# kohjingyu/gill

Hardware: AMD Instinct MI355X
Metric: 512x512 images/sec/node, OPT-6.7B+SD1.5 50-step (higher is better)
Workload: dtype bf16

## Files before the change

### gill_amd/_native.py

```python
from __future__ import annotations

import ctypes as C
import os
from typing import Dict, Iterable, List, Optional, Sequence, Tuple

import torch

_HERE = os.path.dirname(os.path.abspath(__file__))
LIB_PATH = os.environ.get("GILL_AMD_LIB") or os.path.join(_HERE, "libgill_amd.so")


class GillNativeError(RuntimeError):
  pass


class gill_tensor(C.Structure):
  _fields_ = [("name", C.c_char_p), ("data", C.c_void_p), ("dtype", C.c_int32), ("ndim", C.c_int32),
              ("shape", C.c_int64 * 4)]


class gill_opt_config(C.Structure):
  _fields_ = [(n, C.c_int32) for n in ("vocab_size", "hidden_size", "num_layers", "num_heads", "ffn_dim",
                                       "max_positions", "max_batch", "max_seq")]


class gill_mapper_config(C.Structure):
  _fields_ = [(n, C.c_int32) for n in ("in_dim", "out_dim", "hidden_dim", "num_heads", "ffn_dim", "num_enc_layers",
                                       "num_dec_layers", "num_input_tokens", "num_output_tokens", "max_batch")]


class gill_unet_config(C.Structure):
  _fields_ = [("in_channels", C.c_int32), ("out_channels", C.c_int32), ("block_out_channels", C.c_int32 * 4),
              ("layers_per_block", C.c_int32), ("cross_attention_dim", C.c_int32), ("num_heads", C.c_int32),
              ("norm_num_groups", C.c_int32), ("sample_size", C.c_int32), ("ctx_len", C.c_int32),
              ("max_batch", C.c_int32), ("heads_per_level", C.c_int32 * 4), ("v_prediction", C.c_int32),
              ("fp8_convs", C.c_int32)]


class gill_decode_rule(C.Structure):
  _fields_ = [("n_ret", C.c_int32), ("ret_ids", C.c_int32 * 16), ("n_gen", C.c_int32), ("gen_ids", C.c_int32 * 16),
              ("step", C.c_int32), ("min_word_tokens", C.c_int32), ("ret_eq_gen", C.c_int32),
              ("ret_scale", C.c_double), ("gen_scale", C.c_double), ("filter_value", C.c_double)]


class gill_decode_sampler(C.Structure):
  _fields_ = [("seed", C.c_uint64), ("draw", C.c_int32), ("row0", C.c_int32), ("temperature", C.c_double), ("top_p", C.c_double)]


class gill_clip_config(C.Structure):
  _fields_ = [(n, C.c_int32) for n in ("image_size", "patch_size", "hidden_size", "num_layers", "num_heads", "intermediate_size",
                                       "max_batch")]


class gill_clip_text_config(C.Structure):
  _fields_ = [(n, C.c_int32) for n in ("vocab_size", "hidden_size", "num_layers", "num_heads", "intermediate_size", "max_positions",
                                       "hidden_act", "max_batch")]


class gill_vae_config(C.Structure):
  _fields_ = [("latent_channels", C.c_int32), ("out_channels", C.c_int32), ("block_out_channels", C.c_int32 * 4),
              ("layers_per_block", C.c_int32), ("norm_num_groups", C.c_int32), ("latent_size", C.c_int32),
              ("scaling_factor", C.c_float), ("max_batch", C.c_int32)]


class gill_sd_sampler(C.Structure):
  _fields_ = [("kind", C.c_int32), ("steps_offset", C.c_int32), ("set_alpha_to_one", C.c_int32), ("eta", C.c_float)]


SD_ROW_DOUBLES = 12


_vp, _i, _f = C.c_void_p, C.c_int, C.c_float
SYMBOLS: Dict[str, Tuple[object, List[object]]] = {
  "gill_last_error": (C.c_char_p, []),
  "gill_version": (_i, []),
  "gill_opt_create": (_i, [C.POINTER(_vp), C.POINTER(gill_opt_config), C.POINTER(gill_tensor), _i]),
  "gill_opt_destroy": (None, [_vp]),
  "gill_opt_create_ex": (_i, [C.POINTER(_vp), C.POINTER(gill_opt_config), C.POINTER(gill_tensor), _i, _i]),
  "gill_opt_weight_mode": (_i, [_vp]),
  "gill_opt_decode_uses_w8": (_i, [_vp, _i]),
  "gill_opt_cached_uses_w8": (_i, [_vp, _i, _i, _i]),
  "gill_w8_max_rows": (_i, []),
  "gill_op_w8_quant": (_i, [_vp, _i, _i, _vp, _vp, _vp]),
  "gill_op_w8_dequant": (_i, [_vp, _vp, _i, _i, _i, _vp, _vp]),
  "gill_op_linear_w8": (_i, [_vp, _vp, _vp, _vp, _vp, _vp, _i, _i, _i, _i, _i, _i, _vp, _vp, _vp, _vp]),
  "gill_opt_embed": (_i, [_vp, _vp, _i, _vp, _vp]),
  "gill_opt_forward": (_i, [_vp, _vp, _i, _i, _vp, _vp]),
  "gill_opt_forward_cached": (_i, [_vp, _vp, _i, _i, _i, _vp, _vp]),
  "gill_opt_img_hidden": (_i, [_vp, _vp, C.POINTER(C.c_int32), _i, _i, _i, _vp, _vp, _vp]),
  "gill_opt_img_hidden_ex": (_i, [_vp, _vp, C.POINTER(C.c_int32), _i, _i, _i, _vp, _i, _vp, _vp, _vp]),
  "gill_opt_last_logits": (_i, [_vp, _vp, _i, _i, _vp, _vp]),
  "gill_opt_next_token": (_i, [_vp, _vp, _i, _i, C.POINTER(gill_decode_rule), _vp, _vp, _i, _i, _vp, _vp, _vp]),
  "gill_opt_pick_token": (_i, [_vp, _vp, _i, C.POINTER(gill_decode_rule), _vp, _i, _i, _vp, _vp, _vp]),
  "gill_opt_decode_logits": (_i, [_vp, _vp, _i, _i, C.POINTER(gill_decode_rule), _vp, _vp]),
  "gill_opt_filter_logits": (_i, [_vp, _vp, _vp, _i, C.c_double, C.c_double, C.c_double, _i, _vp]),
  "gill_opt_sample_token": (_i, [_vp, _vp, _i, _i, C.POINTER(gill_decode_rule), C.POINTER(gill_decode_sampler), _vp, _vp, _i, _i, _vp,
                                 _vp, _vp]),
  "gill_opt_draw_token": (_i, [_vp, _vp, _i, C.POINTER(gill_decode_rule), C.POINTER(gill_decode_sampler), _vp, _i, _i, _vp, _vp, _vp]),
  "gill_decode_uniforms": (_i, [C.c_uint64, C.c_int32, C.c_int32, C.c_int32, C.c_int32, C.POINTER(C.c_float)]),
  "gill_attention_decode": (_i, [_vp, _vp, _vp, _i, _vp, _vp, _vp, _vp, _i, _i, _i, _i, _vp, _vp]),
  "gill_attention_append": (_i, [_vp, _vp, _vp, _i, _vp, _vp, _vp, _vp, _i, _i, _i, _i, _i, _vp, _vp]),
  "gill_attention_extend": (_i, [_vp, _vp, _vp, _i, _vp, _vp, _vp, _vp, _vp, _i, _i, _i, _i, _i, _i, _vp, _vp]),
  "gill_opt_extend": (_i, [_vp, _vp, _vp, _vp, _i, _vp, _vp, _i, _i, _i, _i, _vp, _vp, _vp]),
  "gill_attention_fork_ws_bytes": (C.c_int64, [_i, _i, _i, _i]),
  "gill_attention_fork": (_i, [_vp, _vp, _vp, _i, _vp, _vp, _vp, _vp, _vp, _vp, _i, _i, _i, _i, _i, _i, _i, _vp, _vp, C.c_int64, _vp]),
  "gill_opt_score_candidates": (_i, [_vp, _vp, _vp, _vp, _i, _vp, _vp, _vp, _vp, _i, _i, _i, _i, _vp, _vp, _vp, _vp, _vp, _vp, _vp, _vp]),
  "gill_opt_set_kv_format": (_i, [_vp, _i]),
  "gill_opt_kv_format": (_i, [_vp]),
  "gill_opt_kv_bytes": (C.c_int64, [_vp]),
  "gill_attention_decode_kv8": (_i, [_vp, _vp, _vp, _i, _vp, _vp, _vp, _vp, _vp, _vp, _i, _i, _i, _i, _vp, _vp]),
  "gill_attention_extend_kv8": (_i, [_vp, _vp, _vp, _i, _vp, _vp, _vp, _vp, _vp, _vp, _vp, _i, _i, _i, _i, _i, _i, _vp, _vp]),
  "gill_opt_decode_step": (_i, [_vp, _vp, _vp, _i, _i, _vp, _vp]),
  "gill_opt_prefill_ids": (_i, [_vp, _vp, _i, _i, _vp, _i, _vp, _vp]),
  "gill_opt_next_token_ragged": (_i, [_vp, _vp, _i, C.POINTER(gill_decode_rule), _i, C.POINTER(gill_decode_sampler), _vp, _vp, _vp, _i, _vp,
                                      _vp]),
  "gill_opt_pick_token_ragged": (_i, [_vp, _vp, _i, C.POINTER(gill_decode_rule), _i, C.POINTER(gill_decode_sampler), _vp, _vp, _i, _vp, _vp]),
  "gill_clip_create": (_i, [C.POINTER(_vp), C.POINTER(gill_clip_config), C.POINTER(gill_tensor), _i]),
  "gill_clip_destroy": (None, [_vp]),
  "gill_clip_forward": (_i, [_vp, _vp, _i, _vp, _vp]),
  "gill_clip_preprocess_workspace": (_i, [C.POINTER(C.c_int64), _i, _i, C.POINTER(C.c_int64)]),
  "gill_clip_preprocess": (_i, [_vp, C.c_int64, C.POINTER(C.c_int64), _i, _i, _i, _vp, _vp, _vp, C.c_int64, _vp]),
  "gill_clip_resize_ksize": (_i, [_i, _i]),
  "gill_clip_resize_taps": (_i, [_i, _i, _i, _i, C.POINTER(C.c_int32), C.POINTER(C.c_int32), C.POINTER(C.c_int32), _i]),
  "gill_clip_text_create": (_i, [C.POINTER(_vp), C.POINTER(gill_clip_text_config), C.POINTER(gill_tensor), _i]),
  "gill_clip_text_destroy": (None, [_vp]),
  "gill_clip_text_forward": (_i, [_vp, _vp, _i, _i, _vp, _vp, _vp]),
  "gill_mapper_create": (_i, [C.POINTER(_vp), C.POINTER(gill_mapper_config), C.POINTER(gill_tensor), _i]),
  "gill_mapper_destroy": (None, [_vp]),
  "gill_mapper_forward": (_i, [_vp, _vp, _vp, _i, _i, _vp, _vp]),
  "gill_unet_create": (_i, [C.POINTER(_vp), C.POINTER(gill_unet_config), C.POINTER(gill_tensor), _i]),
  "gill_unet_destroy": (None, [_vp]),
  "gill_unet_forward": (_i, [_vp, _vp, C.POINTER(C.c_float), _vp, _i, _vp, _vp]),
  "gill_sd_denoise": (_i, [_vp, _vp, _vp, _i, _vp, _i, _i, _f, _vp, _vp]),
  "gill_vae_create": (_i, [C.POINTER(_vp), C.POINTER(gill_vae_config), C.POINTER(gill_tensor), _i]),
  "gill_vae_destroy": (None, [_vp]),
  "gill_vae_decode": (_i, [_vp, _vp, _i, _vp, _vp, _vp]),
  "gill_vae_encode": (_i, [_vp, _vp, _i, _vp, _vp, _vp, _vp]),
  "gill_sd_schedule_from": (_i, [_vp, _i, _i, _i, C.POINTER(C.c_float), C.POINTER(C.c_double), C.POINTER(C.c_double),
                                 C.POINTER(C.c_double)]),
  "gill_sd_denoise_from": (_i, [_vp, _vp, _vp, _vp, _i, _i, _vp, _vp, _i, _i, _f, _vp, _vp, _vp]),
  "gill_op_sd_sampler_run_from": (_i, [_vp, _i, _i, _i, _f, _vp, _vp, _vp, _vp, _i, C.c_int64, _vp, _vp, _vp]),
  "gill_sd_inpaint_prepare": (_i, [_vp, _vp, _i, _i, _i, _i, _vp, _vp, _vp]),
  "gill_sd_inpaint_keep": (_i, [_vp, _i, _i, _i, C.POINTER(C.c_double)]),
  "gill_sd_inpaint": (_i, [_vp, _vp, _vp, _vp, _i, _i, _vp, _vp, _vp, _vp, _i, _i, _f, _vp, _vp, _vp]),
  "gill_op_sd_inpaint_run": (_i, [_vp, _i, _i, _i, _f, _vp, _vp, _vp, _vp, _vp, _vp, _i, C.c_int64, C.c_int64, _vp, _vp, _vp]),
  "gill_op_conv3x3_ex": (_i, [_vp, _i, _vp, _i, _vp, _vp, _vp, _vp, _vp, _i, _i, _i, _i, _i, _i, _i, _i, _vp]),
  "gill_op_conv3x3_fp8": (_i, [_vp, _vp, _vp, _vp, _vp, _i, _i, _i, _i, _i, _i, _vp]),
  "gill_ret_index_create": (_i, [C.POINTER(_vp), _i, C.c_int64]),
  "gill_ret_index_destroy": (None, [_vp]),
  "gill_ret_index_add": (_i, [_vp, _vp, _i, C.c_int64, _i, _f, _vp]),
  "gill_ret_index_size": (C.c_int64, [_vp]),
  "gill_ret_index_rows": (_i, [_vp, C.c_int64, C.c_int64, _vp, _vp]),
  "gill_ret_index_search": (_i, [_vp, _vp, _i, _i, _i, _vp, _i, _f, _vp, _vp, _vp]),
  "gill_ret_index_slabs": (_i, [_vp, C.POINTER(C.c_int64), C.POINTER(C.c_int), C.POINTER(C.c_int64)]),
  "gill_pndm_schedule": (_i, [_i, C.POINTER(C.c_int32), C.POINTER(C.c_double)]),
  "gill_sd_denoise_ex": (_i, [_vp, _vp, _vp, _vp, _i, _vp, _i, _i, _f, _vp, _vp, _vp]),
  "gill_sd_schedule": (_i, [_vp, _i, _i, C.POINTER(C.c_float), C.POINTER(C.c_double), C.POINTER(C.c_double)]),
  "gill_op_sd_sampler_run": (_i, [_vp, _i, _i, _f, _vp, _vp, _vp, _i, C.c_int64, _vp, _vp, _vp]),
  "gill_coop_timeouts": (_i, []),
  "gill_op_gemm": (_i, [_vp, _vp, _vp, _vp, _vp, _i, _i, _i, _f, _i, _i, _i, _vp]),
  "gill_op_geglu": (_i, [_vp, _vp, _vp, _vp, _i, _i, _i, _vp]),
  "gill_op_conv3x3": (_i, [_vp, _i, _vp, _i, _vp, _vp, _vp, _vp, _vp, _i, _i, _i, _i, _i, _i, _i, _vp]),
  "gill_op_attention": (_i, [_vp, _vp, _vp, _vp, _i, _i, _i, _i, _i, _f, _i, _vp]),
  "gill_op_layernorm": (_i, [_vp, _i, _vp, _vp, _vp, _i, _i, _f, _vp]),
  "gill_op_groupnorm": (_i, [_vp, _i, _vp, _i, _i, _i, _i, _vp, _vp, _f, _i, _vp, _vp]),
  "gill_op_conv3x3_gn_stats": (_i, [_vp, _i, _vp, _i, _vp, _vp, _vp, _vp, _vp, _i, _vp, _i, _vp, _vp, _vp, _i, _i, _i, _i, _i, _i, _i,
                                    C.POINTER(C.c_int), C.POINTER(C.c_int), _vp]),
  "gill_op_gemm_gn_stats": (_i, [_vp, _vp, _vp, _vp, _vp, _vp, _i, _i, _i, _i, _i, _i, _i, C.POINTER(C.c_int), C.POINTER(C.c_int), _vp]),
  "gill_op_groupnorm_from_stats": (_i, [_vp, _i, _vp, _i, _i, _i, _i, _vp, _vp, _f, _i, _vp, _i, _i, _vp, _i, _i, _vp, _vp, _f, _vp]),
  "gill_op_conv3x3_gn": (_i, [_vp, _vp, _vp, _vp, _vp, _vp, _vp, _i, _f, _i, _vp, _vp, _vp, _i, _i, _i, _i, _i, _i, _i, _vp]),
  "gill_op_conv3x3_shortcut": (_i, [_vp, _i, _vp, _i, _vp, _vp, _vp, _i, _vp, _i, _vp, _vp, _i, _i, _i, _i, _i, _vp]),
  "gill_op_ffn_fused": (_i, [_vp, _vp, _vp, _vp, _vp, _vp, _vp, _vp, _vp, _vp, _vp, _vp, _i, _i, _vp, _vp, _vp, _vp]),
  "gill_op_geglu_fp8": (_i, [_vp, _vp, _vp, _vp, _vp, _vp, _i, _i, _i, _vp]),
  "gill_conv_fp8_kpad": (_i, [_i]),
  "gill_op_quant_fp8": (_i, [_vp, _f, C.c_int64, _vp, _vp]),
  "gill_op_conv_weight_quant_fp8": (_i, [_vp, _i, _i, _i, _f, _vp, _vp, _vp]),
  "gill_op_conv3x3_fp8_q": (_i, [_vp, _vp, _vp, _vp, _vp, _vp, _vp, _vp, _i, _vp, _i, _i, _i, _i, _i, _i, _i, _vp]),
  "gill_op_groupnorm_fp8": (_i, [_vp, _i, _vp, _i, _i, _i, _i, _vp, _vp, _f, _i, _f, _vp, _vp]),
  "gill_op_linear_weight_quant_fp8": (_i, [_vp, _i, _i, _f, _vp, _vp, _vp]),
  "gill_op_ln_quant_fp8": (_i, [_vp, _i, _i, _vp, _i, _i, _f, _f, _vp, _vp]),
  "gill_op_geglu_fp8_q": (_i, [_vp, _vp, _vp, _vp, _vp, _i, _i, _i, _vp]),
  "gill_op_lnproj": (_i, [_i, _vp, _vp, _vp, _vp, _vp, _vp, _vp, _vp, _vp, _vp, _i, _i, _vp]),
  "gill_op_cross_attention_folded": (_i, [_vp, _vp, _vp, _vp, _vp, _vp, _vp, _vp, _vp, _vp, _vp, _i, _i, _i, _i, _i, _i, _vp]),
  "gill_op_linear_rowstats": (_i, [_vp, _vp, _i, _vp, _vp, _vp, _vp, _vp, _i, C.POINTER(C.c_int), _i, _i, _i, _i, _vp]),
  "gill_op_ln_gemm": (_i, [_i, _vp, _vp, _i, _i, _vp, _vp, _vp, _vp, _vp, _vp, _vp, _vp, _i, _i, _i, _i, _i, _i, _i, _i, _vp]),
  "gill_op_vae_attention": (_i, [_vp, _vp, _vp, _vp, _vp, _vp, _vp, _vp, _i, _i, _i, C.POINTER(C.c_int), _vp]),
  "gill_op_row_softmax": (_i, [_vp, _i, _i, _vp]),
  "gill_op_conv_out": (_i, [_vp, _vp, _i, _vp, _vp, _i, _i, _i, _i, _i, _i, C.POINTER(C.c_int), _vp]),
  "gill_op_conv_in": (_i, [_vp, _vp, _i, _vp, _vp, _i, _i, _i, _i, _i, _vp, _i, _vp]),
  "gill_op_conv_in_wide": (_i, [_vp, _vp, _i, _vp, _vp, _i, _i, _i, _i, _i, _vp, _i, _vp]),
  "gill_op_timestep_embed": (_i, [_vp, _i, _i, _vp, _vp]),
  "gill_op_reduce_ln": (_i, [_vp, _i, _i, _i, _vp, _vp, _vp, _vp, _vp, _f, _vp]),
  "gill_op_linear_reduce_ln": (_i, [_vp, _vp, _vp, _vp, _vp, _vp, _vp, _i, _i, _i, _i, _i, _vp]),
  "gill_op_skinny_gemm": (_i, [_vp, _vp, _vp, _i, _i, _i, _vp]),
  "gill_op_lm_head_loss": (_i, [_vp, _vp, _vp, _i, _i, _i, _vp, _vp, _vp, _vp, _vp]),
  "gill_lm_loss_geometry": (_i, [_i, _i, _i, C.POINTER(C.c_int), C.POINTER(C.c_int), C.POINTER(C.c_int), C.POINTER(C.c_int)]),
  "gill_op_img_block_heads": (_i, [_vp, C.c_int64, _i, _vp, _i, _vp, _vp, _i, _vp, _vp, _i, _vp, _vp, _vp, _vp]),
  "gill_op_img_rerank_scores": (_i, [_vp, _vp, _i, _i, _i, _vp, _vp]),
  "gill_gemm_plan": (_i, [_vp, _i, _i, _i, _i, _vp]),
  "gill_gemm_plan_log": (_i, [_vp, _i, C.POINTER(C.c_int)]),
  "gill_unet_xf_plan": (_i, [_vp, _i, _i, _i, _i, _vp]),
  "gill_gemm_query": (_i, [_vp, _i, _i, _i, _i, _vp]),
  "gill_attention_plan": (_i, [_i, _i, _i, _i, _i, _i, _i, _vp]),
  "gill_opt_forward_loss": (_i, [_vp, _vp, C.POINTER(C.c_int32), _i, _i, _i, _vp, _i, _vp, _vp, _vp, _vp, _vp, _vp, _vp, _vp, _vp]),
}

_lib: Optional[C.CDLL] = None


def lib() -> C.CDLL:
  global _lib
  if _lib is None:
    if not os.path.exists(LIB_PATH):
      raise GillNativeError(
        f"{LIB_PATH} is missing: the HIP extension is the only implementation of the GILL hot path. "
        "Build it with `python -c 'import __graft_entry__ as g; g.build()'` (or `make -C gill_amd/csrc`).")
    l = C.CDLL(LIB_PATH)
    for name, (res, args) in SYMBOLS.items():
      fn = getattr(l, name)
      fn.restype = res
      fn.argtypes = args
    _lib = l
  return _lib


def check(rc: int) -> None:
  if rc != 0:
    msg = lib().gill_last_error()
    raise GillNativeError(f"libgill_amd error {rc}: {msg.decode() if msg else '?'}")


def current_stream() -> int:
  return int(torch.cuda.current_stream().cuda_stream)


_DTYPES = {torch.bfloat16: 0, torch.float32: 1, torch.float16: 2}


def ptr(t: Optional[torch.Tensor]) -> Optional[int]:
  if t is None:
    return None
  assert t.is_cuda and t.is_contiguous(), "libgill_amd takes contiguous device tensors"
  return t.data_ptr()


def make_tensor_table(state: Dict[str, torch.Tensor], device: torch.device):
  keep = []
  arr = (gill_tensor * len(state))()
  for i, (k, v) in enumerate(state.items()):
    if v.dtype not in _DTYPES:
      v = v.float()
    v = v.detach().to(device).contiguous()
    name = k.encode()
    keep.append((name, v))
    arr[i].name = name
    arr[i].data = v.data_ptr()
    arr[i].dtype = _DTYPES[v.dtype]
    arr[i].ndim = v.dim()
    for d in range(4):
      arr[i].shape[d] = v.shape[d] if d < v.dim() else 1
  return arr, keep
```

### gill_amd/csrc/ffn.hip

```cpp
#include "ops.h"
#include <type_traits>

namespace {

constexpr int FC = 320;
constexpr int FH = 1280;
constexpr int FTM = 128;
constexpr int FSLOT = 20 * 1024;
constexpr int FNSLOT = 7;
constexpr int FNCH = FH / 64;
constexpr int FBIAS_OFF = FNSLOT * FSLOT;
constexpr int FBO2_OFF = FBIAS_OFF + FNCH * 128 * 4;
constexpr int FW_BYTES = 2560;
constexpr int FSMEM = FBIAS_OFF + FNCH * 128 * 4;
constexpr int FSMEM_PRE = FBO2_OFF + FC * 4;
static_assert(FSMEM_PRE <= 160 * 1024, "LDS budget");
constexpr int FKO = 384;
constexpr int FNPRE = 2 * (FKO / 64);

typedef __attribute__((ext_vector_type(16))) float f32x16;
typedef __attribute__((ext_vector_type(4))) float f32x4;
typedef __attribute__((ext_vector_type(4))) unsigned u32x4;
typedef __attribute__((ext_vector_type(2))) unsigned u32x2;

template <int N> __device__ __forceinline__ void ffn_wait_vm() {
  __builtin_amdgcn_s_waitcnt((N & 15) | ((N >> 4) << 14) | (7 << 4) | (15 << 8));
}

struct Slab { const bf16_t* src; int ld; };

template <bool PRE>
__global__ __launch_bounds__(256) __attribute__((amdgpu_waves_per_eu(1, 1))) void ffn_fused_kernel(const FfnArgs p) {
  kernarg_warm<sizeof(FfnArgs)>();
  constexpr int SB = PRE ? FNPRE % 7 : 0;
  extern __shared__ __attribute__((aligned(16))) unsigned char smem[];
  const int tid = threadIdx.x, lane = tid & 63;
  const int w = __builtin_amdgcn_readfirstlane(tid >> 6);
  const int l31 = lane & 31, hi = lane >> 5;
  const int m = blockIdx.x * FTM + w * 32 + l31;

  const int srow = lane >> 3, schunk = (lane & 7) ^ srow;
  auto slab_f = [&](int f) -> Slab {
    if constexpr (PRE) return Slab{p.Wpp + (size_t)(f / 5) * 160 * FC + 64 * (f % 5), FC};
    else return Slab{p.Wfo + (size_t)(f / 5) * 160 * (5 * FC) + 4 * FC + 64 * (f % 5), 5 * FC};
  };
  auto slab_g = [&](int g) -> Slab { return Slab{p.Wo + (size_t)(g / 6) * 160 * FKO + 64 * (g % 6), FKO}; };
  auto slab_c = [&](int c, int q) -> Slab {
    if (q < 5) return Slab{p.W1c + (size_t)c * 128 * FC + 64 * q, FC};
    return Slab{p.W2p + (size_t)(q - 5) * 160 * FH + 64 * c, FH};
  };
  auto issue_piece = [&](const Slab& st, int slot, int i) {
    const int pc = w + 4 * i;
    const uint64_t b64 = (uint64_t)(uintptr_t)(st.src + (size_t)(8 * pc) * st.ld);
    const bf16_t* base = (const bf16_t*)(uintptr_t)(((uint64_t)(unsigned)__builtin_amdgcn_readfirstlane((unsigned)(b64 >> 32)) << 32) |
                                                     (uint64_t)(unsigned)__builtin_amdgcn_readfirstlane((unsigned)b64));
    const bf16_t* src = (const bf16_t*)((const char*)base + (unsigned)((srow * st.ld + schunk * 8) * 2));
    __builtin_amdgcn_global_load_lds((const __attribute__((address_space(1))) void*)src,
                                     (__attribute__((address_space(3))) void*)(smem + slot * FSLOT + pc * 1024), 16, 0, 0);
  };
  auto wfrag = [&](const unsigned char* slot, int tile, int s) -> bf16x8 {
    const int row = tile * 32 + l31;
    return *reinterpret_cast<const bf16x8*>(slot + row * 128 + (((2 * s + hi) ^ (row & 7)) * 16));
  };

#pragma unroll
  for (int f = 0; f < 6; ++f) {
    const Slab st = PRE ? slab_g(f) : slab_f(f);
#pragma unroll
    for (int i = 0; i < 5; ++i) issue_piece(st, f, i);
  }
  __builtin_amdgcn_sched_barrier(0);
  bf16x8 tf[20];
  float ln_mean, ln_rstd;
  bf16x8 xf[PRE ? FKO / 16 : 1];
  u32x4 res[PRE ? 20 : 1];
  if constexpr (PRE) {
    const bf16_t* tsrc = p.T + (size_t)(blockIdx.x * FTM + w * 32 + (lane >> 2)) * FC + (lane & 3) * 8;
#pragma unroll
    for (int i = 0; i < 10; ++i) {
      res[2 * i] = *reinterpret_cast<const u32x4*>(tsrc + 32 * i);
      res[2 * i + 1] = *reinterpret_cast<const u32x4*>(tsrc + 32 * i + 16 * FC);
    }
#pragma unroll
    for (int s = 0; s < FKO / 16; ++s) xf[s] = *reinterpret_cast<const bf16x8*>(p.X + (size_t)m * FKO + 16 * s + 8 * hi);
  } else {
#pragma unroll
    for (int s = 0; s < 20; ++s) tf[s] = *reinterpret_cast<const bf16x8*>(p.T + (size_t)m * FC + 16 * s + 8 * hi);
    const int R = p.ln_rows ? p.ln_rows : p.M;
    const int mr = m >= R ? m - R : m;
    const float* base = p.ln_stats + (size_t)mr * 2;
    const size_t pstride = (size_t)R * 2;
    float2 st = make_float2(0.f, 0.f);
    for (int pl = 0; pl < p.ln_planes; ++pl) {
      const float2 v = *reinterpret_cast<const float2*>(base + (size_t)pl * pstride);
      st.x += v.x; st.y += v.y;
    }
    ln_mean = st.x * (1.f / FC);
    const float var = fmaxf(st.y * (1.f / FC) - ln_mean * ln_mean, 0.f);
    ln_rstd = rsqrtf(var + p.ln_eps);
  }
  {
    float* bt = reinterpret_cast<float*>(smem + FBIAS_OFF);
    static_assert(FNCH * 128 % 256 == 0, "table fill: whole rounds of the workgroup");
    float tb[FNCH * 128 / 256];
#pragma unroll
    for (int j = 0; j < FNCH * 128 / 256; ++j) tb[j] = p.b1c[tid + 256 * j];
#pragma unroll
    for (int j = 0; j < FNCH * 128 / 256; ++j) bt[tid + 256 * j] = tb[j];
    if constexpr (PRE) {
      float* b2t = reinterpret_cast<float*>(smem + FBO2_OFF);
      const float v0 = p.bo2[tid], v1 = p.bo2[min(tid + 256, FC - 1)];
      b2t[tid] = v0; b2t[min(tid + 256, FC - 1)] = v1;
    }
  }

  ffn_wait_vm<0>();

  bf16x8 wf[2][5];
  auto run_stage = [&](auto ntile_tag, auto ntile_next_tag, auto wait_tag, auto nxp_tag, int slot_idx, int next_slot_idx, const Slab& nx,
                       int nx_slot, auto&& mma, auto phase_end_tag) {
    constexpr bool PHASE_END = decltype(phase_end_tag)::value;
    constexpr int NTL = decltype(ntile_tag)::value;
    constexpr int NTN = decltype(ntile_next_tag)::value;
    constexpr int WAITN = decltype(wait_tag)::value;
    constexpr int NXP = decltype(nxp_tag)::value;
    const unsigned char* slot = smem + slot_idx * FSLOT;
    const unsigned char* nslot = smem + next_slot_idx * FSLOT;
#pragma unroll
    for (int s = 0; s < 4; ++s) {
      __builtin_amdgcn_sched_barrier(0);
      if (s == 3 && NTN > 0) {
        ffn_wait_vm<WAITN>();
        __builtin_amdgcn_s_barrier();
        __builtin_amdgcn_sched_barrier(0);
      }
      if (s + 1 < 4) {
#pragma unroll
        for (int q = 0; q < NTL; ++q) wf[(s + 1) & 1][q] = wfrag(slot, q, s + 1);
      } else if (NTN > 0 && !PHASE_END) {
#pragma unroll
        for (int q = 0; q < NTN; ++q) wf[0][q] = wfrag(nslot, q, 0);
      }
      if (NXP > 0) { issue_piece(nx, nx_slot, s); if (s == 3 && NXP == 5) issue_piece(nx, nx_slot, 4); }
      mma(s, wf[s & 1]);
#pragma unroll
      for (int q = 0; q < NTL; ++q) {
        __builtin_amdgcn_sched_group_barrier(0x008, 1, 0);
        if (q == 0 && (s + 1 < 4 || (NTN > 0 && !PHASE_END))) __builtin_amdgcn_sched_group_barrier(0x100, 5, 0);
        __builtin_amdgcn_sched_group_barrier(0x006, 3, 0);
        if (q == 2 && NXP > 0) __builtin_amdgcn_sched_group_barrier(0x020, 1, 0);
        if (q == 3 && NXP == 5 && s == 3) __builtin_amdgcn_sched_group_barrier(0x020, 1, 0);
      }
    }
  };
  using I4 = std::integral_constant<int, 4>; using I5 = std::integral_constant<int, 5>;

  __builtin_amdgcn_s_waitcnt(0xC07F);
  __builtin_amdgcn_s_barrier();
#pragma unroll
  for (int q = 0; q < 5; ++q) wf[0][q] = wfrag(smem, q, 0);

  if constexpr (PRE) {
    f32x16 acc1[10];
    {
      unsigned char* wb = smem + 6 * FSLOT + w * FW_BYTES;
      const float* b2t = reinterpret_cast<const float*>(smem + FBO2_OFF);
      const unsigned wb_wr = (unsigned)(uintptr_t)(__attribute__((address_space(3))) unsigned char*)wb + (lane >> 2) * 80 + (lane & 3) * 16;
#pragma unroll
      for (int i = 0; i < 10; ++i) {
        asm volatile("ds_write_b128 %0, %1\n\tds_write_b128 %0, %2 offset:1280" ::"v"(wb_wr), "v"(res[2 * i]), "v"(res[2 * i + 1]) : "memory");
#pragma unroll
        for (int q4 = 0; q4 < 4; ++q4) {
          const f32x4 bv = *reinterpret_cast<const f32x4*>(b2t + 32 * i + 8 * q4 + 4 * hi);
          const u32x2 r = *reinterpret_cast<const u32x2*>(wb + l31 * 80 + q4 * 16 + hi * 8);
          acc1[i][4 * q4] = bv.x + __uint_as_float(r.x << 16);
          acc1[i][4 * q4 + 1] = bv.y + __uint_as_float(r.x & 0xffff0000u);
          acc1[i][4 * q4 + 2] = bv.z + __uint_as_float(r.y << 16);
          acc1[i][4 * q4 + 3] = bv.w + __uint_as_float(r.y & 0xffff0000u);
        }
      }
    }
    __builtin_amdgcn_s_waitcnt(0xC07F);
    __builtin_amdgcn_s_barrier();
    __builtin_amdgcn_sched_barrier(0);
#define G_STAGE(G)                                                                                                               \
    {                                                                                                                            \
      auto mma = [&](int s, const bf16x8* wfp) {                                                                                 \
        _Pragma("unroll") for (int q = 0; q < 5; ++q)                                                                           \
          acc1[5 * ((G) / 6) + q] = __builtin_amdgcn_mfma_f32_32x32x16_bf16(wfp[q], xf[4 * ((G) % 6) + s], acc1[5 * ((G) / 6) + q], 0, 0, 0); \
      };                                                                                                                         \
      const Slab nx = (G) + 6 < FNPRE ? slab_g((G) + 6) : slab_f((G) + 6 - FNPRE);                                               \
      run_stage(I5{}, I5{}, std::integral_constant<int, 23>{}, I5{}, (G) % 7, ((G) + 1) % 7, nx, ((G) + 6) % 7, mma,             \
                std::integral_constant<bool, (G) + 1 == FNPRE>{});                                                               \
    }
    G_STAGE(0) G_STAGE(1) G_STAGE(2) G_STAGE(3) G_STAGE(4) G_STAGE(5) G_STAGE(6) G_STAGE(7) G_STAGE(8) G_STAGE(9) G_STAGE(10) G_STAGE(11)
#undef G_STAGE
    float sum = 0.f, sq = 0.f;
#pragma unroll
    for (int i = 0; i < 10; ++i)
#pragma unroll
      for (int hh = 0; hh < 2; ++hh) {
        union { bf16x8 v; unsigned u[4]; } pk;
#pragma unroll
        for (int jj = 0; jj < 4; ++jj) {
          const unsigned o = pack_bf2(acc1[i][8 * hh + 2 * jj], acc1[i][8 * hh + 2 * jj + 1]);
          const float v0 = __uint_as_float(o << 16), v1 = __uint_as_float(o & 0xffff0000u);
          sum += v0 + v1;
          sq += v0 * v0 + v1 * v1;
          pk.u[jj] = o;
        }
        tf[2 * i + hh] = pk.v;
      }
    sum += __shfl_xor(sum, 32, 64);
    sq += __shfl_xor(sq, 32, 64);
    ln_mean = sum * (1.f / FC);
    ln_rstd = rsqrtf(fmaxf(sq * (1.f / FC) - ln_mean * ln_mean, 0.f) + p.ln_eps);
#pragma unroll
    for (int q = 0; q < 5; ++q) wf[0][q] = wfrag(smem + (SB % 7) * FSLOT, q, 0);
  }

  __builtin_amdgcn_sched_barrier(0);
  f32x16 out[10];
#pragma unroll
  for (int i = 0; i < 10; ++i)
#pragma unroll
    for (int r = 0; r < 16; ++r) out[i][r] = 0.f;

#define F_STAGE(F, N)                                                                                                            \
  {                                                                                                                              \
    auto mma = [&](int s, const bf16x8* wfp) {                                                                                   \
      _Pragma("unroll") for (int q = 0; q < 5; ++q)                                                                             \
        out[5 * ((F) / 5) + q] = __builtin_amdgcn_mfma_f32_32x32x16_bf16(wfp[q], tf[4 * ((F) % 5) + s], out[5 * ((F) / 5) + q], 0, 0, 0); \
    };                                                                                                                           \
    const Slab nx = (F) + 6 < 10 ? slab_f(((F) + 6) % 10) : slab_c(0, ((F) + 6 - 10) % 7);                                       \
    run_stage(I5{}, std::integral_constant<int, (F) + 1 < 10 ? 5 : 4>{}, std::integral_constant<int, N>{},                       \
              std::integral_constant<int, ((F) + 6 < 10 || (F) + 6 - 10 >= 5) ? 5 : 4>{}, (SB + (F)) % 7, (SB + (F) + 1) % 7, nx,            \
              (SB + (F) + 6) % 7, mma, std::false_type{});                                                                                               \
  }
  F_STAGE(0, 23) F_STAGE(1, 23) F_STAGE(2, 23) F_STAGE(3, 23) F_STAGE(4, 23)
  F_STAGE(5, 22) F_STAGE(6, 21) F_STAGE(7, 20) F_STAGE(8, 19) F_STAGE(9, 19)
#undef F_STAGE

#pragma unroll
  for (int s = 0; s < 20; ++s) {
    union { bf16x8 v; unsigned u[4]; } x;
    x.v = tf[s];
#pragma unroll
    for (int j = 0; j < 4; ++j) {
      if constexpr (PRE) asm volatile("" : "+v"(x.u[j]));
      const float a = (__uint_as_float(x.u[j] << 16) - ln_mean) * ln_rstd;
      const float b = (__uint_as_float(x.u[j] & 0xffff0000u) - ln_mean) * ln_rstd;
      x.u[j] = pack_bf2(a, b);
    }
    tf[s] = x.v;
  }
  const float* btab = reinterpret_cast<const float*>(smem + FBIAS_OFF);

  auto run_chunk = [&](int c, auto last_tag) {
    constexpr bool LAST = decltype(last_tag)::value;
    f32x16 acc[4];
#pragma unroll
    for (int i = 0; i < 4; ++i)
#pragma unroll
      for (int r = 0; r < 16; ++r) acc[i][r] = 0.f;
#define S1_STAGE(J, N, NL)                                                                                                      \
    {                                                                                                                            \
      auto mma = [&](int s, const bf16x8* wfp) {                                                                                 \
        _Pragma("unroll") for (int nt = 0; nt < 4; ++nt)                                                                        \
          acc[nt] = __builtin_amdgcn_mfma_f32_32x32x16_bf16(wfp[nt], tf[4 * (J) + s], acc[nt], 0, 0, 0);                         \
      };                                                                                                                         \
      const Slab nx = (J) == 0 ? slab_c(c, 6) : slab_c(LAST ? c : c + 1, (J) - 1);                                               \
      run_stage(I4{}, std::integral_constant<int, (J) == 4 ? 5 : 4>{}, std::integral_constant<int, LAST ? NL : N>{},             \
                std::integral_constant<int, (J) == 0 ? 5 : (LAST ? 0 : 4)>{}, (SB + 3 + (J)) % 7, (SB + 4 + (J)) % 7, nx,        \
                (SB + 2 + (J)) % 7, mma, std::false_type{});                                                                     \
    }
    S1_STAGE(0, 20, 20) S1_STAGE(1, 21, 18) S1_STAGE(2, 21, 14) S1_STAGE(3, 21, 10) S1_STAGE(4, 20, 5)
#undef S1_STAGE
    bf16x8 pf[4];
#pragma unroll
    for (int tt = 0; tt < 2; ++tt)
#pragma unroll
      for (int hh = 0; hh < 2; ++hh) {
        union { bf16x8 v; unsigned u[4]; } pk;
#pragma unroll
        for (int g2 = 0; g2 < 2; ++g2) {
          const f32x4 bv = *reinterpret_cast<const f32x4*>(btab + c * 128 + tt * 32 + 16 * hh + 8 * g2 + 4 * hi);
          const f32x4 bg = *reinterpret_cast<const f32x4*>(btab + c * 128 + 64 + tt * 32 + 16 * hh + 8 * g2 + 4 * hi);
          const int r = 8 * hh + 4 * g2;
          const float o0 = (acc[tt][r] + bv.x) * gelu_logistic(acc[2 + tt][r] + bg.x);
          const float o1 = (acc[tt][r + 1] + bv.y) * gelu_logistic(acc[2 + tt][r + 1] + bg.y);
          const float o2 = (acc[tt][r + 2] + bv.z) * gelu_logistic(acc[2 + tt][r + 2] + bg.z);
          const float o3 = (acc[tt][r + 3] + bv.w) * gelu_logistic(acc[2 + tt][r + 3] + bg.w);
          pk.u[2 * g2] = pack_bf2(o0, o1);
          pk.u[2 * g2 + 1] = pack_bf2(o2, o3);
        }
        pf[2 * tt + hh] = pk.v;
      }
#define S2_STAGE(U, N, NL)                                                                                                      \
    {                                                                                                                            \
      auto mma = [&](int s, const bf16x8* wfp) {                                                                                 \
        _Pragma("unroll") for (int q = 0; q < 5; ++q)                                                                           \
          out[5 * (U) + q] = __builtin_amdgcn_mfma_f32_32x32x16_bf16(wfp[q], pf[s], out[5 * (U) + q], 0, 0, 0);                  \
      };                                                                                                                         \
      const Slab nx = slab_c(LAST ? c : c + 1, 4 + (U));                                                                         \
      run_stage(I5{}, std::integral_constant<int, (U) == 0 ? 5 : (LAST ? 0 : 4)>{}, std::integral_constant<int, LAST ? NL : N>{},\
                std::integral_constant<int, LAST ? 0 : ((U) == 1 ? 5 : 4)>{}, (SB + 8 + (U)) % 7, (SB + 9 + (U)) % 7, nx,        \
                (SB + 7 + (U)) % 7, mma, std::false_type{});                                                                     \
    }
    S2_STAGE(0, 19, 0) S2_STAGE(1, 19, 0)
#undef S2_STAGE
  };
  for (int c = 0; c + 1 < FNCH; ++c) run_chunk(c, std::false_type{});
  run_chunk(FNCH - 1, std::true_type{});

  constexpr int OSTR = 656;
  __syncthreads();
  unsigned char* wtile = smem + (size_t)(w * 32) * OSTR;
  unsigned char* otile = wtile + (size_t)l31 * OSTR;
  {
    const bf16_t* rsrc = p.resid + (size_t)(blockIdx.x * FTM + w * 32) * FC;
    u32x4 rr[20];
#pragma unroll
    for (int j = 0; j < 20; ++j) rr[j] = *reinterpret_cast<const u32x4*>(rsrc + (size_t)(lane + 64 * j) * 8);
#pragma unroll
    for (int j = 0; j < 20; ++j) {
      const int c = lane + 64 * j;
      *reinterpret_cast<u32x4*>(wtile + (c / 40) * OSTR + (c % 40) * 16) = rr[j];
    }
  }
#pragma unroll
  for (int i = 0; i < 10; ++i) {
#pragma unroll
    for (int q4 = 0; q4 < 4; ++q4) {
      const int n = i * 32 + 8 * q4 + 4 * hi;
      const f32x4 bo = *reinterpret_cast<const f32x4*>(p.bo + n);
      const u32x2 rv = *reinterpret_cast<const u32x2*>(otile + n * 2);
      const float v0 = out[i][4 * q4] + bo.x + __uint_as_float(rv.x << 16);
      const float v1 = out[i][4 * q4 + 1] + bo.y + __uint_as_float(rv.x & 0xffff0000u);
      const float v2 = out[i][4 * q4 + 2] + bo.z + __uint_as_float(rv.y << 16);
      const float v3 = out[i][4 * q4 + 3] + bo.w + __uint_as_float(rv.y & 0xffff0000u);
      *reinterpret_cast<u32x2*>(otile + n * 2) = u32x2{pack_bf2(v0, v1), pack_bf2(v2, v3)};
    }
  }
  {
    bf16_t* odst = p.out + (size_t)(blockIdx.x * FTM + w * 32) * FC;
#pragma unroll
    for (int j = 0; j < 20; ++j) {
      const int c = lane + 64 * j;
      *reinterpret_cast<u32x4*>(odst + (size_t)c * 8) = *reinterpret_cast<const u32x4*>(wtile + (c / 40) * OSTR + (c % 40) * 16);
    }
  }
  if (p.gn_stats) {
    __syncthreads();
    float2* colsum = reinterpret_cast<float2*>(smem + 128 * OSTR);
    for (int idx = tid; idx < 2 * FC; idx += 256) {
      const int slab = idx / FC, col = idx - slab * FC;
      const unsigned char* src = smem + (size_t)(slab * 64) * OSTR + col * 2;
      float a = 0.f, q = 0.f;
#pragma unroll 8
      for (int r = 0; r < 64; ++r) {
        const float v = __uint_as_float((unsigned)*reinterpret_cast<const unsigned short*>(src + (size_t)r * OSTR) << 16);
        a += v; q += v * v;
      }
      colsum[idx] = make_float2(a, q);
    }
    __syncthreads();
    {
      const int which = tid & 1, bin = (tid >> 1) & 63, slab = tid >> 7;
      const float* cs = reinterpret_cast<const float*>(colsum + slab * FC + bin * 5) + which;
      const float a = (((cs[0] + cs[2]) + cs[4]) + cs[6]) + cs[8];
      const int m0 = blockIdx.x * FTM + slab * 64;
      const int b = m0 / p.rows_per_batch;
      const int sl = (m0 - b * p.rows_per_batch) / 64;
      const int nslab = p.rows_per_batch / 64;
      p.gn_stats[(((size_t)b * nslab + sl) * 64 + bin) * 2 + which] = a;
    }
  }
}

__global__ __launch_bounds__(256) void ffn_relayout_kernel(const bf16_t* __restrict__ wff1, const float* __restrict__ bff1,
                                                           const bf16_t* __restrict__ wfo, bf16_t* __restrict__ W1c,
                                                           float* __restrict__ b1c, bf16_t* __restrict__ W2p, bf16_t* __restrict__ Wpp) {
  const int64_t n1 = (int64_t)2 * FH * FC, n2 = (int64_t)FC * FH, n3 = Wpp ? (int64_t)FC * FC : 0;
  auto perm16 = [](int pos) { const int g16 = pos / 16, r = pos % 16, hi = r / 8, j = r % 8; return 16 * g16 + 8 * (j >> 2) + 4 * hi + (j & 3); };
  for (int64_t i = (int64_t)blockIdx.x * blockDim.x + threadIdx.x; i < n1 + n2 + n3; i += (int64_t)gridDim.x * blockDim.x) {
    if (i < n1) {
      const int k = (int)(i % FC);
      const int row = (int)(i / FC);
      const int c = row / 128, rr = row % 128, gate = rr / 64, j = rr % 64;
      const int h = c * 64 + j;
      const int src = (h / 16) * 32 + gate * 16 + (h % 16);
      W1c[i] = wff1[(size_t)src * FC + (Wpp ? perm16(k) : k)];
      if (k == 0) b1c[row] = bff1[src];
    } else if (i < n1 + n2) {
      const int64_t t = i - n1;
      const int pos = (int)(t % FH), n = (int)(t / FH);
      W2p[t] = wfo[(size_t)n * (5 * FC) + perm16(pos)];
    } else {
      const int64_t t = i - n1 - n2;
      const int pos = (int)(t % FC), n = (int)(t / FC);
      Wpp[t] = wfo[(size_t)n * (5 * FC) + 4 * FC + perm16(pos)];
    }
  }
}

}

bool ffn_fused_supported(int C, int M) { return C == FC && M % FTM == 0 && M > 0; }

int ffn_relayout_launch(const bf16_t* wff1, const float* bff1, const bf16_t* wfo, bf16_t* W1c, float* b1c, bf16_t* W2p, bf16_t* Wpp,
                        hipStream_t s) {
  hipLaunchKernelGGL(ffn_relayout_kernel, dim3(1024), dim3(256), 0, s, wff1, bff1, wfo, W1c, b1c, W2p, Wpp);
  GILL_CHECK_HIP(hipGetLastError());
  return 0;
}

int ffn_fused_launch(const FfnArgs& a, hipStream_t s) {
  GILL_REQUIRE(ffn_fused_supported(FC, a.M), "fused feed-forward block: M must be a multiple of 128");
  GILL_REQUIRE(a.T && a.W1c && a.b1c && a.W2p && a.bo && a.resid && a.out, "fused feed-forward block: null operand");
  GILL_REQUIRE(!a.gn_stats || (a.rows_per_batch > 0 && a.rows_per_batch % 128 == 0), "fused feed-forward block: GroupNorm partials need whole 64-row slabs per sample");
  const bool pre = a.X != nullptr;
  if (pre) {
    GILL_REQUIRE(a.Wo && a.bo2 && a.Wpp, "fused feed-forward block with attn2.to_out in front: null operand");
  } else {
    GILL_REQUIRE(a.Wfo && a.ln_stats && a.ln_planes >= 1, "fused feed-forward block: LayerNorm row-sum planes missing");
  }
  static bool attr_set[2] = {false, false};
  const void* fn = pre ? (const void*)ffn_fused_kernel<true> : (const void*)ffn_fused_kernel<false>;
  const int smem = pre ? FSMEM_PRE : FSMEM;
  if (!attr_set[pre]) {
    GILL_CHECK_HIP(hipFuncSetAttribute(fn, hipFuncAttributeMaxDynamicSharedMemorySize, smem));
    attr_set[pre] = true;
  }
  if (pre) hipLaunchKernelGGL(ffn_fused_kernel<true>, dim3(a.M / FTM), dim3(256), smem, s, a);
  else hipLaunchKernelGGL(ffn_fused_kernel<false>, dim3(a.M / FTM), dim3(256), smem, s, a);
  GILL_CHECK_HIP(hipGetLastError());
  return 0;
}
```

### gill_amd/csrc/ops.h

```cpp
#pragma once
#include "common.h"

enum { ACT_NONE = 0, ACT_RELU = 1, ACT_GELU = 2, ACT_SILU = 3, ACT_GEGLU = 4, ACT_QUICK_GELU = 5  };
enum { OUT_BF16 = 0, OUT_F32 = 1, OUT_QKV = 2, OUT_SOFTMAX80 = 3 };

struct GemmArgs {
  int M = 0, N = 0, K = 0;
  const bf16_t* A = nullptr;  int lda = 0;
  const bf16_t* A2 = nullptr; int lda2 = 0;
  int K1 = 0;
  int conv = 0;
  int IH = 0, IW = 0, OH = 0, OW = 0, Cin = 0, stride = 1, ups = 0;
  int pad_shift = 0;
  const bf16_t* X1 = nullptr; const bf16_t* X2 = nullptr; int KX = 0, KX1 = 0;
  const bf16_t* W = nullptr;
  int k_chunked = 0;
  float alpha = 1.f;
  const float* bias = nullptr;
  const float* rowvec = nullptr; int rows_per_batch = 1; int rowvec_bstride = 0;
  const void* resid = nullptr; int ldr = 0; int resid_f32 = 0;
  int act = ACT_NONE;
  int out_mode = OUT_BF16;
  void* C = nullptr; int ldc = 0;
  bf16_t* Cq = nullptr; bf16_t* Ck = nullptr; bf16_t* Cvt = nullptr;
  int heads = 0, dp = 0, dpv = 0, ntok = 0, ntok_pad_q = 0, ntok_pad_kv = 0, seg_base = 0;
  float qscale = 1.f;
  int kv_tok_offset = 0;
  int splitk = 1; float* ws = nullptr;
  int w_blk64 = 0;
  int partials_only = 0;
  float* gn_stats = nullptr; int gn_groups = 0; int gn_cg = 0;
  float* row_stats = nullptr;
  const float* ln_stats = nullptr; int ln_planes = 1; int ln_rows = 0; const float* ln_colsum = nullptr; float ln_eps = 1e-5f;
  int wb_rows = 0; int64_t wb_stride = 0; int vb_stride = 0;
  bf16_t* fn_Y = nullptr; const float* fn_gamma = nullptr; const float* fn_beta = nullptr; float fn_eps = 1e-5f; int fn_silu = 0; int fn_cg = 0;
  unsigned* coop_ctr = nullptr; float* fn_ss = nullptr;
  int spare_word = 0;
};
bool gemm_coop_ok(const GemmArgs& a);
int gemm_coop_counters(const GemmArgs& a);
int gemm_coop_giveups(unsigned* count);
int gemm_coop_mode();
bool gemm_fused_norm_ok(const GemmArgs& a);
int gemm_launch(const GemmArgs& a, hipStream_t s);
#define GN_SLAB_ROWS 64
#define GN_SLAB_ROWS_MIN 16
int gemm_gn_slab_rows(const GemmArgs& a);
#define GEMM_MAX_ROW_PLANES(N) (((N) + 63) / 64 > 2 * (((N) + 127) / 128) ? ((N) + 63) / 64 : 2 * (((N) + 127) / 128))
int gemm_row_planes(const GemmArgs& a);
bool gemm_fused_gn_ok(int N, int cg);
int gemm_pick_splitk(int M, int N, int K, int act, bool plain = false, bool generic = false);
#ifndef GEMM_STREAM64_MAX_ROWS
#define GEMM_STREAM64_MAX_ROWS 256
#endif
bool gemm_stream64_weights(int N, int K);
int gemm_pick_splitk_blk64(int M, int N, int K);

int gemm_splitk_reduce_launch(const GemmArgs& a, hipStream_t s);

#define F8_ACT_SCALE 8.0f
struct ConvF8Args {
  int B = 0, H = 0, W = 0, Cin = 0, M = 0, N = 0, Kpad = 0;
  const unsigned char* A8 = nullptr;
  const unsigned char* W8 = nullptr;
  const float* colscale = nullptr;
  const float* bias = nullptr;
  const float* rowvec = nullptr; int rows_per_batch = 1; int rowvec_bstride = 0;
  const bf16_t* resid = nullptr;
  bf16_t* C = nullptr;
  float* gn_stats = nullptr; int gn_groups = 0; int gn_cg = 0;
  int splitk = 1; float* ws = nullptr;
};
int conv3x3_fp8_launch(const ConvF8Args& a, hipStream_t s);

#define F8_LIN_ACT_SCALE 16.0f
struct LinF8Args {
  int M = 0, N = 0, K = 0;
  const unsigned char* A8 = nullptr;
  const unsigned char* W8 = nullptr;
  const float* colscale = nullptr;
  const float* bias = nullptr;
  bf16_t* C = nullptr;
};
int geglu_fp8_launch(const LinF8Args& a, hipStream_t s);
int linear_weight_quant_fp8_launch(const bf16_t* w, int N, int K, float act_scale, unsigned char* w8, float* colscale, hipStream_t s);
int ln_quant_fp8_launch(const bf16_t* t, int M, int C, const float* ln_stats, int planes, int ln_rows, float eps, float act_scale, unsigned char* y,
                        hipStream_t s);
int conv_fp8_kpad(int Cin);
int quant_bf16_fp8_launch(const bf16_t* x, float scale, int64_t n, unsigned char* y, hipStream_t s);
int conv_weight_quant_fp8_launch(const void* w_oihw, int dtype, int Cout, int Cin, float act_scale, unsigned char* w8, float* colscale,
                                 hipStream_t s);

struct AttnArgs {
  const bf16_t* Q = nullptr; const bf16_t* K = nullptr; const bf16_t* Vt = nullptr; bf16_t* O = nullptr;
  int B = 0, H = 0, nq = 0, nkv = 0, nq_pad = 0, nkv_pad = 0, dp = 0, dpv = 0;
  int ldo = 0;
  float scale = 1.f;
  int d = 0;
  int causal = 0;
  int kv_bstride_zero = 0;
  int xcd_map = 1;
};
int attention_launch(const AttnArgs& a, hipStream_t s);

struct AttnDecodeArgs {
  const bf16_t* q = nullptr; const bf16_t* k = nullptr; const bf16_t* v = nullptr; int ld = 0;
  bf16_t* K = nullptr; bf16_t* Vt = nullptr;
  const int32_t* lens = nullptr;
  bf16_t* O = nullptr; int ldo = 0;
  int32_t* flags = nullptr;
  int B = 0, H = 0, dp = 0, dpv = 0, pitch = 0;
  float qscale = 1.f;
};
int attention_decode_launch(const AttnDecodeArgs& a, hipStream_t s);

struct AttnAppendArgs : AttnDecodeArgs {
  int nq = 1;
};
int attention_append_launch(const AttnAppendArgs& a, hipStream_t s);

struct AttnExtendArgs : AttnDecodeArgs {
  const int32_t* cu_new = nullptr;
  int total_new = 0, max_new = 0;
};
int attention_extend_launch(const AttnExtendArgs& a, hipStream_t s);

struct AttnDecodeKv8Args {
  const bf16_t* q = nullptr; const bf16_t* k = nullptr; const bf16_t* v = nullptr; int ld = 0;
  uint8_t* K8 = nullptr; uint8_t* Vt8 = nullptr; int8_t* Kexp = nullptr; int8_t* Vexp = nullptr;
  const int32_t* lens = nullptr;
  bf16_t* O = nullptr; int ldo = 0;
  int32_t* flags = nullptr;
  int B = 0, H = 0, dp = 0, dpv = 0, pitch = 0;
  float qscale = 1.f;
};
int attention_decode_kv8_launch(const AttnDecodeKv8Args& a, hipStream_t s);
struct AttnExtendKv8Args : AttnDecodeKv8Args {
  const int32_t* cu_new = nullptr;
  int total_new = 0, max_new = 0;
};
int attention_extend_kv8_launch(const AttnExtendKv8Args& a, hipStream_t s);

struct AttnForkArgs {
  const bf16_t* q = nullptr; const bf16_t* k = nullptr; const bf16_t* v = nullptr; int ld = 0;
  const bf16_t* K = nullptr; const bf16_t* Vt = nullptr;
  const int32_t* parent = nullptr; const int32_t* plen = nullptr; const int32_t* cu_new = nullptr;
  bf16_t* O = nullptr; int ldo = 0;
  int32_t* flags = nullptr;
  int C = 0, Bc = 0, H = 0, dp = 0, dpv = 0, pitch = 0, total_new = 0, max_new = 0;
  float qscale = 1.f;
  void* ws = nullptr; size_t ws_bytes = 0;
};
size_t attention_fork_ws_bytes(int C, int H, int d, int max_new);
int attention_fork_launch(const AttnForkArgs& a, hipStream_t s);


struct FfnArgs {
  int M = 0;
  const bf16_t* T = nullptr;
  const float* ln_stats = nullptr; int ln_planes = 0, ln_rows = 0; float ln_eps = 1e-5f;
  const bf16_t* W1c = nullptr; const float* b1c = nullptr;
  const bf16_t* W2p = nullptr;
  const bf16_t* Wfo = nullptr; const float* bo = nullptr;
  const bf16_t* resid = nullptr; bf16_t* out = nullptr;
  float* gn_stats = nullptr; int rows_per_batch = 0;
  const bf16_t* X = nullptr;
  const bf16_t* Wo = nullptr; const float* bo2 = nullptr;
  const bf16_t* Wpp = nullptr;
};
bool ffn_fused_supported(int C, int M);
int ffn_relayout_launch(const bf16_t* wff1, const float* bff1, const bf16_t* wfo, bf16_t* W1c, float* b1c, bf16_t* W2p, bf16_t* Wpp,
                        hipStream_t s);
int ffn_fused_launch(const FfnArgs& a, hipStream_t s);

struct LnProjArgs {
  int mode = 0;
  int M = 0;
  const bf16_t* X = nullptr;
  bf16_t* T = nullptr;
  const bf16_t* W1 = nullptr;
  const float* b1 = nullptr;
  const bf16_t* W2p = nullptr;
  const float* c2 = nullptr;
  float ln_eps = 1e-5f;
  bf16_t *Cq = nullptr, *Ck = nullptr, *Cvt = nullptr;
  int heads = 0, dp = 0, dpv = 0, ntok = 0, ntok_pad = 0, seg_base = 0;
  float qscale = 1.f;
  const float* gn_ss = nullptr;
};
bool lnproj_supported(int C, int M, int heads, int dp);
int lnproj_kperm_launch(const bf16_t* src, int N, bf16_t* dst, hipStream_t s);
int lnproj_launch(const LnProjArgs& a, hipStream_t s);

int layernorm_launch(const void* x, int x_f32, const float* gamma, const float* beta, bf16_t* y,
                     int rows, int C, float eps, hipStream_t s);
int layernorm_f32out_launch(const void* x, int x_f32, const float* gamma, const float* beta, float* y,
                            int rows, int C, float eps, hipStream_t s);

#define GN_STATS_ROWS 32
static inline size_t groupnorm_stats_floats(int B, int HW, int groups) {
  return (size_t)B * ((HW + GN_STATS_ROWS - 1) / GN_STATS_ROWS) * groups * 2 + (size_t)B * groups * 2;
}
static inline size_t groupnorm_totals_floats(int B, int nbins1, int nbins2) { return (size_t)B * (nbins1 + nbins2) * 2; }
int groupnorm_launch(const bf16_t* x1, int C1, const bf16_t* x2, int C2, int B, int HW, int groups,
                     const float* gamma, const float* beta, float eps, int silu, bf16_t* y,
                     float* stats, hipStream_t s, float out8_scale = 0.f);
int groupnorm_apply_launch(const bf16_t* x1, int C1, const bf16_t* x2, int C2, int B, int HW, int groups, const float* gamma,
                           const float* beta, float eps, int silu, bf16_t* y, const float* stats1, int bin1, int sc1, int nslab1,
                           const float* stats2, int bin2, int nslab2, hipStream_t s, float out8_scale = 0.f,
                           float* tot_scratch = nullptr, float* ss_out = nullptr);
bool groupnorm_bins_align(int cg, int sc1, int bin1, int bin2);

int embed_rows_bf16_launch(const int64_t* ids, const bf16_t* table, int vocab, int n, int D, bf16_t* out, hipStream_t s);
int embed_tokens_launch(const int64_t* ids, const bf16_t* table, int vocab, const bf16_t* extra, int n_extra, const bf16_t* pos_table,
                        int pos_offset, int B, int T, int D, float* out_f32, hipStream_t s);
int gather_rows_launch(const void* src, int src_f32, const int32_t* row_idx, int nrows, int D, void* dst, int dst_f32,
                       hipStream_t s);
int add_cast_launch(const void* a, int a_f32, const void* b, int b_f32, int64_t n, int64_t b_period, bf16_t* out,
                    hipStream_t s);
int cast_f32_to_bf16_launch(const float* x, bf16_t* y, int64_t n, hipStream_t s);
int cast_bf16_to_f32_launch(const bf16_t* x, float* y, int64_t n, hipStream_t s);
int timestep_embed_launch(const float* t, int n, int dim, bf16_t* out, hipStream_t s);
int silu_bf16_launch(const bf16_t* x, bf16_t* y, int64_t n, hipStream_t s);
int im2col_nchw_launch(const float* x, int B, int Cin, int H, int W, int kpad, bf16_t* out, hipStream_t s, unsigned* zero = nullptr, int nzero = 0);
int conv_out_launch(const bf16_t* x, const bf16_t* w , const float* bias, int B, int Cin, int H, int W,
                    int Cout, float* y, hipStream_t s, int force_general = 0, int* path = nullptr);
int skinny_gemm_launch(const bf16_t* x, const bf16_t* W, int M, int N, int K, float* out, hipStream_t s);
void lm_loss_geometry(int M, int V, int D, int* row_tile, int* col_tile, int* n_slabs, int* cols_per_slab);
size_t lm_loss_workspace_bytes(int M, int V);
int lm_loss_launch(const bf16_t* X, const bf16_t* W, const int64_t* target, int M, int V, int D, float* lse, float* tgt, int* rank, float* summary,
                   void* workspace, hipStream_t s);
int img_heads_launch(const float* hidden, int64_t rows, int D, const int* row_idx, int n, const bf16_t* Wr, const float* br, int E, const bf16_t* Wd,
                     const float* bd, int C, float* ret_emb, float* probs, int* choice, hipStream_t s);
int img_rerank_launch(const float* visual, const float* ret_emb, int n, int g, int E, float* scores, hipStream_t s);
constexpr int kDecodeMaxIds = 16;
struct DecodeRuleDev {
  int vocab;
  int n_ret, n_gen;
  int ret[kDecodeMaxIds], gen[kDecodeMaxIds];
  int64_t ret_raw[kDecodeMaxIds];
  int64_t ret0_raw;
  int special;
  int suppress;
  int do_ret_scale, do_gen_scale;
  float ret_scale, gen_scale, filter_value;
  int ret_eq_gen;
};
int decode_rule_pick_launch(float* logits, int B, int V, const DecodeRuleDev& r, const bf16_t* table, int D, int64_t* tokens,
                            int ld, int col, int32_t* n_out, bf16_t* next_embeds, hipStream_t s);
int decode_rule_launch(float* logits, int B, int V, const DecodeRuleDev& r, hipStream_t s);
struct DecodeSampler {
  uint64_t seed;
  int draw, row0;
  double temperature, top_p;
};
int decode_sample_check(int B, int V, const DecodeRuleDev& r, const DecodeSampler& sm, int D, int ld, int col);
int decode_sample_launch(float* logits, int B, int V, const DecodeRuleDev& r, const DecodeSampler& sm, const bf16_t* table, int D,
                         int64_t* tokens, int ld, int col, int32_t* n_out, bf16_t* next_embeds, hipStream_t s);
enum { DEC_LEN = 0, DEC_STEP = 1, DEC_FORCED = 2, DEC_NTOK = 3, DEC_ROW_ID = 4, DEC_FLAGS = 5, DEC_FIELDS = 6 };
enum { DEC_FLAG_ASSERT = 1, DEC_FLAG_CLAMP = 2, DEC_FLAG_FULL = 4 };
int decode_ragged_launch(float* logits, int B, int V, const DecodeRuleDev& r, int min_word_tokens, int max_steps, const DecodeSampler* sm,
                         int32_t* state, int32_t* clamp_flags, const bf16_t* table, int D, int64_t* tokens, int ld, bf16_t* next_embeds,
                         hipStream_t s);
int decode_filter_launch(const float* in, float* out, int B, int V, double temperature, int reciprocal, double top_p,
                         double filter_value, hipStream_t s);
struct PlmsRow {
  int mode;
  int slot_new;
  int s1, s2, s3;
  float sample_coeff, eps_coeff;
};
struct SamplerRow {
  int slot_new, s1;
  float in_scale;
  float p_x, p_e;
  float c_x, c_0, c_1, c_n;
};
struct SdLoopArgs {
  const PlmsRow* rows;
  const SamplerRow* srows = nullptr;
  const float* const* noise = nullptr;
  int* ctr;
  const float* temb_table; int temb_total;
  float* temb_cur;
  const float* eps;
  float* lat;
  float* lat2;
  float* cur_sample;
  float* ets;
  int B; int64_t n;
  const float* guidance;
  int cfg;
};
int zero_bytes_launch(void* dst, size_t bytes, hipStream_t s);
int copy_bytes_launch(void* dst, const void* src, size_t bytes, hipStream_t s);
int dup_pair_launch(void* a, const void* b, void* b2, size_t bytes, hipStream_t s);
int sd_stage_launch(const SdLoopArgs& a, hipStream_t s);
int plms_step_launch(const SdLoopArgs& a, hipStream_t s);
int sampler_step_launch(const SdLoopArgs& a, hipStream_t s);
int scale_f32_launch(const float* src, float scale, int64_t n, float* dst, hipStream_t s);
int add_noise_f32_launch(const float* x, const float* z, float a, float b, int64_t n, float* dst, hipStream_t s);
struct SdInpaintArgs {
  SdLoopArgs l;
  const float* x0 = nullptr;
  const float* z0 = nullptr;
  const float* mask = nullptr;
  const float* xm = nullptr;
  const float* keep = nullptr;
  int64_t hw = 0;
};
int inpaint_prepare_launch(const float* image, const float* mask, int B, int Bm, int H, int W, float* masked, float* lmask, hipStream_t s);
int sd_blend_launch(const SdInpaintArgs& a, hipStream_t s);
int sd_stage_concat_launch(const SdInpaintArgs& a, hipStream_t s);

int conv_weight_relayout_launch(const void* w, int dtype, int Cout, int Cin, bf16_t* out , hipStream_t s);
bool gemm_conv_pingpong(int rows_multiple_of, int Cout);
bool conv_k_chunked(int HW, int Cin, int Cout);
int conv_weight_relayout_ups4_launch(const void* w, int dtype, int Cout, int Cin, bf16_t* out , hipStream_t s);
int conv_weight_relayout_chunked_launch(const void* w, int dtype, int Cout, int Cin, bf16_t* out , hipStream_t s);
int convert_to_bf16_launch(const void* src, int dtype, int64_t n, bf16_t* dst, hipStream_t s);
int convert_to_bf16_blk64_launch(const void* src, int dtype, int N, int K, bf16_t* dst, hipStream_t s);
int convert_to_f32_launch(const void* src, int dtype, int64_t n, float* dst, hipStream_t s);
// ... 42 lines not shown
```

### gill_amd/csrc/unet.hip

```cpp
#include "convnet.h"
#include "sd_schedule.h"
#include "xf_weights.h"
#include "xf_plan.h"
#include "xf_args.h"
#include <math.h>
#include <map>
#include <set>

namespace {

struct LinW { bf16_t* w = nullptr; float* b = nullptr; int out = 0, in = 0; };

struct ResnetW : ResW {
  LinW sc;
  int temb_off = 0;
};

struct XfW {
  int C = 0, heads = 0, d = 0, dp = 0, dpv = 0, layer_id = 0;
  XfGeom geom{};
  XfForms forms{};
  NormW gn;
  LinW proj_in, proj_out;
  NormW ln1, ln2, ln3;
// ... 349 lines not shown
      Tensor y; bool has_y = false; const float* ss = nullptr;
      const Tensor* copy() const { return has_y ? &y : nullptr; }
    };
    FusedNorm* offer(const NormW& n, float eps, int silu, int H, int W, int C, bool table = false) {
      Tensor y; y.H = H; y.W = W; y.C = C;
      if (!table) y = r.talloc(H, W, C);
      fn = FusedNorm{&n, eps, silu, y, true, false};
      if (table) fn.ss = (float*)r.m->arena.alloc(sizeof(float) * (size_t)r.Bx * 2 * C);
      return &fn;
    }
    Taken take() {
      Taken t;
      if (fn.done && fn.ss) t.ss = fn.ss;
      else if (fn.done) { t.y = fn.y; t.has_y = true; }
      fn.done = false;
      return t;
    }
  };
  int gemm(GemmArgs& g, RowStats* rs = nullptr, Tensor* ys = nullptr, FusedNorm* fn = nullptr) {
    unsigned* ctr = dry ? nullptr : m->coop_ctr + m->coop_next;
    m->coop_next += (size_t)gemm_coop_counters(g);
    if (dry) return 0;
    GILL_REQUIRE(m->coop_next <= m->coop_n, "internal: COOP counter pool exhausted");
    pick_sk(g);
    if (g.out_mode == OUT_SOFTMAX80 || (g.wb_rows && g.wb_rows % 128 != 0)) g.splitk = 1;
    g.coop_ctr = ctr;
    if (fn) {
      g.rows_per_batch = fn->y.H * fn->y.W;
      g.fn_Y = fn->ss ? nullptr : fn->y.p; g.fn_ss = fn->ss;
      g.fn_gamma = fn->n->g; g.fn_beta = fn->n->b; g.fn_eps = fn->eps; g.fn_silu = fn->silu;
      g.fn_cg = g.N / m->cfg.norm_num_groups;
      if (gemm_coop_ok(g) || (g.splitk > 1 && !fn->ss && gemm_fused_norm_ok(g))) {
        fn->done = true;
        if (!fn->raw_needed) {
          g.C = nullptr;
          if (g.splitk > 1) { g.gn_stats = nullptr; if (ys) ys->stats = nullptr; }
        }
      } else {
        g.fn_Y = nullptr; g.fn_ss = nullptr;
      }
    }
    if (rs) { g.row_stats = rs->p; rs->planes = gemm_row_planes(g); }
    if (ys && ys->stats) ys->nslab = ys->H * ys->W / gemm_gn_slab_rows(g);
    GILL_TRY(gemm_launch(g, s));
    return dbg_sync(g.conv ? "conv" : (g.act == ACT_GEGLU ? "geglu" : (g.out_mode == OUT_QKV ? "qkv" : (g.out_mode == OUT_SOFTMAX80 ? "scores+softmax" : "gemm"))), g.M, g.N, g.K);
  }
  int gnorm(const Tensor& x1, const Tensor* x2, const NormW& n, float eps, int silu, const Tensor& y, float y8_scale = 0.f,
            float* ss_out = nullptr, bool* folded = nullptr) {
    GILL_TRY(dbg_sync("before groupnorm", x1.C, x2 ? x2->C : 0, x1.H * x1.W));
    return ConvRun::gnorm(x1, x2, n, eps, silu, y, y8_scale, ss_out, folded);
  }
  int conv8(const Tensor& x8, const ConvW& w, const float* rowvec, int rv_bstride, const bf16_t* resid, Tensor& y) {
    if (dry) return 0;
    ConvF8Args a;
    a.B = Bx; a.H = x8.H; a.W = x8.W; a.Cin = w.cin; a.M = Bx * x8.H * x8.W; a.N = w.cout; a.Kpad = w.kpad;
    a.A8 = reinterpret_cast<const unsigned char*>(x8.p); a.W8 = w.w8; a.colscale = w.cs; a.C = y.p;
    a.rows_per_batch = x8.H * x8.W;
    GemmArgs g;
    g.M = a.M; g.N = a.N; g.K = 9 * w.cin;
    pick_sk(g, true);
    a.splitk = g.splitk;
    if (a.splitk > 1) {
      a.ws = g.ws;
      GILL_TRY(conv3x3_fp8_launch(a, s));
      g.bias = w.b; g.rowvec = rowvec; g.rows_per_batch = a.rows_per_batch; g.rowvec_bstride = rv_bstride;
      g.resid = resid; g.ldr = w.cout; g.C = y.p; g.ldc = w.cout;
      fuse_stats(g, y);
      if (y.stats) y.nslab = y.H * y.W / gemm_gn_slab_rows(g);
      return gemm_splitk_reduce_launch(g, s);
    }
    a.bias = w.b; a.rowvec = rowvec; a.rowvec_bstride = rv_bstride; a.resid = resid;
    if (y.stats) { a.gn_stats = y.stats; a.gn_groups = y.C / y.sbin; a.gn_cg = y.sbin; y.nslab = y.H * y.W / GN_SLAB_ROWS; }
    return conv3x3_fp8_launch(a, s);
  }
  int conv(const Tensor& x1, const Tensor* x2, const ConvW& w, int stride, int ups, const float* rowvec, int rv_bstride,
           const bf16_t* resid, Tensor& y, FusedNorm* fn = nullptr) {
    GemmArgs g = conv_args(x1, x2, w, stride, ups, rowvec, rv_bstride, resid, y);
    return gemm(g, nullptr, &y, fn);
  }
  int linear(const bf16_t* A, int lda, const bf16_t* A2, int lda2, int K1, int M, const bf16_t* W, const float* b, int N,
             int K, const bf16_t* resid, int act, bf16_t* out, int ldc, Tensor* ystats = nullptr,
             RowStats* row_stats = nullptr, FusedNorm* fn = nullptr) {
    GemmArgs g;
    g.M = M; g.N = N; g.K = K; g.K1 = K1; g.A = A; g.lda = lda; g.A2 = A2; g.lda2 = lda2; g.W = W; g.bias = b;
    g.resid = resid; g.ldr = N; g.act = act; g.C = out; g.ldc = ldc;
    if (ystats) fuse_stats(g, *ystats);
    return gemm(g, row_stats, ystats, fn);
  }

  int resnet(const Tensor& x1, const Tensor* x2, const ResnetW& w, Tensor* out, bool out_stats, const Tensor* pre = nullptr,
             FusedNorm* next = nullptr) {
    const int H = x1.H, Wd = x1.W;
    *out = talloc(H, Wd, w.cout, out_stats);
    const size_t mk = m->arena.mark();
    if (w.c1.w8) {
      Tensor n1 = talloc8(H, Wd, w.cin);
      GILL_TRY(gnorm(x1, x2, w.n1, 1e-5f, 1, n1, F8_ACT_SCALE));
      Tensor h = talloc(H, Wd, w.cout, true);
      GILL_TRY(conv8(n1, w.c1, temb_rows ? temb_rows + w.temb_off : nullptr, temb_bstride, nullptr, h));
      Tensor n2 = talloc8(H, Wd, w.cout);
      GILL_TRY(gnorm(h, nullptr, w.n2, 1e-5f, 1, n2, F8_ACT_SCALE));
      const bf16_t* resid = x1.p;
      if (w.has_sc) {
        GILL_TRY(linear(x1.p, x1.C, x2 ? x2->p : nullptr, x2 ? x2->C : 0, x1.C, Bx * H * Wd, w.sc.w, w.sc.b, w.cout, w.cin, nullptr, 0,
                        out->p, w.cout));
        resid = out->p;
      }
      GILL_TRY(conv8(n2, w.c2, nullptr, 0, resid, *out));
      m->arena.release(mk);
      return 0;
    }
    Tensor n1 = talloc(H, Wd, w.cin);
    if (pre && !x2) n1 = *pre;
    else GILL_TRY(gnorm(x1, x2, w.n1, 1e-5f, 1, n1));
    Tensor h = talloc(H, Wd, w.cout, true);
    Tensor n2 = talloc(H, Wd, w.cout);
    FusedNorm f2{&w.n2, 1e-5f, 1, n2, false, false};
    GILL_TRY(conv(n1, nullptr, w.c1, 1, 0, temb_rows ? temb_rows + w.temb_off : nullptr, temb_bstride, nullptr, h, &f2));
    if (!f2.done) GILL_TRY(gnorm(h, nullptr, w.n2, 1e-5f, 1, n2));
    if (w.has_sc) {
      GemmArgs g = conv2_shortcut_args(n2, x1, x2, w, *out);
      GILL_TRY(gemm(g, nullptr, out, next));
    } else {
      GILL_TRY(conv(n2, nullptr, w.c2, 1, 0, nullptr, 0, x1.p, *out, next));
    }
    m->arena.release(mk);
    return 0;
  }

  int attend(const bf16_t* q, const bf16_t* k, const bf16_t* vt, bf16_t* o, int nq, int nkv, int nq_pad, int nkv_pad,
             const XfW& w) {
    if (dry) return 0;
    AttnArgs a;
    a.Q = q; a.K = k; a.Vt = vt; a.O = o;
    a.B = Bx; a.H = w.heads; a.nq = nq; a.nkv = nkv; a.nq_pad = nq_pad; a.nkv_pad = nkv_pad;
    a.dp = w.dp; a.dpv = w.dpv; a.ldo = w.heads * w.dp; a.d = w.d;
    a.scale = 1.0f / sqrtf((float)w.d);
    return attention_launch(a, s);
  }

  struct BatchScope {
    int& Bx; const int saved;
    BatchScope(int& Bx, int b) : Bx(Bx), saved(Bx) { Bx = b; }
    ~BatchScope() { Bx = saved; }
  };
  XfPlan xf_plan_of(const XfW& w, int HW, bool shared) const { return xf_plan(w.forms, w.geom, shared ? 2 * Bx : Bx, HW, shared); }
  struct XfBlock {
    const XfW& w; const XfPlan p; const int HW, hw_pad, Bpre; const bool shared;
    Tensor t;
    Tensor xd;
    bf16_t *q, *k, *vt, *o;
    RowStats st1, st2, st3;
    XfHeads heads() const { return xf_heads(w.heads, w.d); }
    LnProjArgs lnproj_args() const {
      LnProjArgs lp;
      lp.M = p.M; lp.T = t.p; lp.heads = w.heads; lp.dp = w.dp; lp.dpv = w.dpv; lp.ntok = HW; lp.ntok_pad = hw_pad;
      lp.Cq = q; lp.Ck = k; lp.Cvt = vt; lp.qscale = heads().qscale;
      return lp;
    }
  };

  int xf_self_attention(XfBlock& b, const bf16_t* n, const float* gn_ss) {
    const XfW& w = b.w; const int C = w.C;
    if (b.p.lnproj) {
      LnProjArgs lp = b.lnproj_args();
      lp.mode = 0; lp.X = n; lp.gn_ss = gn_ss; lp.W1 = w.proj_in.w; lp.b1 = w.proj_in.b; lp.W2p = w.wqkv1p; lp.c2 = w.c_qkv1;
      if (!dry) GILL_TRY(lnproj_launch(lp, s));
    } else {
      GILL_TRY(linear(n, C, nullptr, 0, C, b.p.M1, w.proj_in.w, w.proj_in.b, C, C, nullptr, ACT_NONE, b.t.p, C, nullptr, &b.st1));
      GemmArgs g = xf_qkv_args(b.t.p, b.p.M1, C, {b.st1.p, b.st1.planes, 0}, w.wqkv1, w.s_qkv1, w.c_qkv1, 3, b.heads(), b.HW, b.q, b.k, b.vt);
      GILL_TRY(gemm(g));
    }
    BatchScope half(Bx, b.Bpre);
    return attend(b.q, b.k, b.vt, b.o, b.HW, b.HW, b.hw_pad, b.hw_pad, w);
  }

  int xf_cross_attention(XfBlock& b, const Tensor& x) {
    const XfW& w = b.w; const XfPlan& p = b.p; const int C = w.C, hdp = w.heads * w.dp;
    if (p.lnproj) {
      LnProjArgs lp = b.lnproj_args();
      lp.mode = 1; lp.X = b.o; lp.W1 = w.out1.w; lp.b1 = w.out1.b; lp.W2p = w.wq2p; lp.c2 = w.c_q2;
      if (!dry) GILL_TRY(lnproj_launch(lp, s));
    } else {
      GILL_TRY(linear(b.o, hdp, nullptr, 0, hdp, p.M1, w.out1.w, w.out1.b, C, hdp, b.t.p, ACT_NONE, b.t.p, C, nullptr, &b.st2));
      if (b.shared && !dry) GILL_TRY(dup_pair_launch(b.t.p, x.p, b.xd.p, sizeof(bf16_t) * (size_t)p.M1 * C, s));
      const XfLnRows ln2 = {b.st2.p, b.st2.planes, p.M1};
      if (p.cross == XF_CROSS_XALG) {
        const int id = w.layer_id;
        GemmArgs g, g2;
        xf_xalg_args(b.t.p, p.M, b.HW, C, w.heads, ln2, m->xq_w[id], m->xq_cs[id], m->xq_b[id], m->xo_w[id], w.out2.b, b.o, b.t.p, b.t.p, &g, &g2);
        GILL_TRY(gemm(g));
        return gemm(g2, &b.st3);
      }
      GemmArgs g = xf_qkv_args(b.t.p, p.M, C, ln2, w.wq2, w.s_q2, w.c_q2, 1, b.heads(), b.HW, b.q, b.k, b.vt);
      GILL_TRY(gemm(g));
    }
    GILL_REQUIRE(m->kcache[w.layer_id] != nullptr || dry, "internal: cross-attention K/V cache missing");
    GILL_TRY(attend(b.q, m->kcache[w.layer_id], m->vcache[w.layer_id], b.o, b.HW, m->cfg.ctx_len, b.hw_pad, m->ctx_pad, w));
    if (p.ffn == XF_FFN_FUSED_PRE) return 0;
    return linear(b.o, hdp, nullptr, 0, hdp, p.M, w.out2.w, w.out2.b, C, hdp, b.t.p, ACT_NONE, b.t.p, C, nullptr, &b.st3);
  }

  int xf_feed_forward(XfBlock& b, Tensor* out, FusedNorm* next) {
    const XfW& w = b.w; const XfPlan& p = b.p; const int C = w.C, M = p.M;
    if (p.ffn == XF_FFN_FUSED || p.ffn == XF_FFN_FUSED_PRE) {
      if (dry) return 0;
      FfnArgs fa;
      fa.M = M; fa.T = b.t.p; fa.ln_stats = b.st3.p; fa.ln_planes = b.st3.planes;
      fa.W1c = w.w1c; fa.b1c = w.b1c; fa.W2p = w.w2p; fa.Wfo = w.wfo; fa.bo = w.bfo; fa.resid = b.xd.p; fa.out = out->p;
      if (p.ffn == XF_FFN_FUSED_PRE) { fa.X = b.o; fa.Wo = w.out2.w; fa.bo2 = w.out2.b; fa.Wpp = w.wpp; }
      if (out->stats && out->sbin == 5) { fa.gn_stats = out->stats; fa.rows_per_batch = b.HW; out->nslab = b.HW / GN_SLAB_ROWS; }
      else out->stats = nullptr;
      return ffn_fused_launch(fa, s);
    }
    bf16_t* ffh = (bf16_t*)m->arena.alloc(sizeof(bf16_t) * (size_t)M * 4 * C);
    if (p.ffn == XF_FFN_GEMM_FP8) {
      unsigned char* t8 = (unsigned char*)m->arena.alloc((size_t)M * C);
      if (!dry) {
        GILL_TRY(ln_quant_fp8_launch(b.t.p, M, C, b.st3.p, b.st3.planes, 0, 1e-5f, F8_LIN_ACT_SCALE, t8, s));
        LinF8Args a;
        a.M = M; a.N = 8 * C; a.K = C; a.A8 = t8; a.W8 = w.wff1_8; a.colscale = w.cs_ff1; a.bias = w.bff1; a.C = ffh;
        GILL_TRY(geglu_fp8_launch(a, s));
        GILL_TRY(dbg_sync("geglu fp8", M, 8 * C, C));
      }
    } else {
      GemmArgs g = xf_geglu_args(b.t.p, M, C, 4 * C, {b.st3.p, b.st3.planes, 0}, w.wff1, w.s_ff1, w.bff1, ffh);
      GILL_TRY(gemm(g));
    }
    return linear(ffh, 4 * C, b.t.p, C, 4 * C, M, w.wfo, w.bfo, C, 5 * C, b.xd.p, ACT_NONE, out->p, C, out, nullptr, next);
  }

  int xf(const Tensor& x, const XfW& w, Tensor* out, bool out_stats, bool shared = false, const Tensor* pre = nullptr,
         FusedNorm* next = nullptr, const float* pre_ss = nullptr) {
    const int H = x.H, Wd = x.W, C = w.C, HW = H * Wd;
    XfBlock b{w, xf_plan_of(w, HW, shared), HW, round_up(HW, 32), Bx, shared};
    BatchScope full(Bx, shared ? 2 * Bx : Bx);
    *out = talloc(H, Wd, C, out_stats);
    const size_t mk = m->arena.mark();
    Tensor n = talloc(H, Wd, C);
    b.xd = shared ? talloc(H, Wd, C) : x;
    float* gn_ss = nullptr;
    bool gn_folded = false;
    {
      BatchScope half(Bx, b.Bpre);
      if (b.p.gn_table) gn_ss = (float*)m->arena.alloc(sizeof(float) * (size_t)Bx * 2 * C);
      if (pre_ss && gn_ss) { gn_ss = const_cast<float*>(pre_ss); gn_folded = true; }
      else if (pre) n = *pre;
      else GILL_TRY(gnorm(x, nullptr, w.gn, 1e-6f, 0, n, 0.f, gn_ss, &gn_folded));
    }
    b.t = talloc(H, Wd, C);
    b.st1 = ln_slot(b.p.M, C); b.st2 = ln_slot(b.p.M, C); b.st3 = ln_slot(b.p.M, C);
    b.q = (bf16_t*)m->arena.alloc(sizeof(bf16_t) * (size_t)Bx * w.heads * b.hw_pad * w.dp);
    b.k = (bf16_t*)m->arena.alloc(sizeof(bf16_t) * (size_t)Bx * w.heads * b.hw_pad * w.dp);
    b.vt = (bf16_t*)m->arena.alloc(sizeof(bf16_t) * (size_t)Bx * w.heads * w.dpv * b.hw_pad);
    b.o = (bf16_t*)m->arena.alloc(sizeof(bf16_t) * (size_t)b.p.M * w.heads * w.dp);
    GILL_TRY(xf_self_attention(b, gn_folded ? x.p : n.p, gn_folded ? gn_ss : nullptr));
    GILL_TRY(xf_cross_attention(b, x));
    GILL_TRY(xf_feed_forward(b, out, next));
    m->arena.release(mk);
    return 0;
  }

  int forward(const float* sample, float* eps_out) {
    const gill_unet_config& c = m->cfg;
    const int* ch = c.block_out_channels;
    const int L = c.sample_size;
    m->arena.off = 0;
    m->gn_next = 0;
    m->ln_next = 0;
    m->coop_next = 0;
    std::vector<Tensor> skips;
    Tensor x = talloc(L, L, ch[0], true);
    {
      const size_t mk = m->arena.mark();
      const int kpad = conv_in_kpad(c.in_channels);
      bf16_t* col = (bf16_t*)m->arena.alloc(sizeof(bf16_t) * (size_t)Bx * L * L * kpad);
      if (!dry) GILL_TRY(im2col_nchw_launch(sample, Bx, c.in_channels, L, L, kpad, col, s, m->coop_ctr, (int)m->coop_n));
      GILL_TRY(linear(col, kpad, nullptr, 0, kpad, Bx * L * L, m->conv_in_w, m->conv_in_b, ch[0], kpad, nullptr, ACT_NONE, x.p, ch[0], &x));
      m->arena.release(mk);
    }
    skips.push_back(x);
    Handoff pn{*this};
    for (int i = 0; i < 4; ++i) {
      for (int j = 0; j < 2; ++j) {
        Tensor y;
        const bool share = cfg_pair && i == 0 && j == 0 && Bx % 2 == 0 && temb_bstride == 0;
        BatchScope prefix(Bx, share ? Bx / 2 : Bx);
        const Handoff::Taken pre = pn.take();
        FusedNorm* nx = nullptr;
        if (i < 3) nx = pn.offer(m->down_xf[i][j].gn, 1e-6f, 0, x.H, x.W, ch[i], xf_plan_of(m->down_xf[i][j], x.H * x.W, share).gn_table);
        else nx = pn.offer(j == 0 ? m->down_res[3][1].n1 : m->mid_res[0].n1, 1e-5f, 1, x.H, x.W, ch[i]);
        GILL_TRY(resnet(x, nullptr, m->down_res[i][j], &y, true, pre.copy(), nx));
        x = y;
        if (i < 3) {
          const Handoff::Taken pre2 = pn.take();
          FusedNorm* nx2 = (i >= 2 && j == 0) ? pn.offer(m->down_res[i][1].n1, 1e-5f, 1, x.H, x.W, ch[i]) : nullptr;
          Tensor z; GILL_TRY(xf(x, m->down_xf[i][j], &z, true, share, pre2.copy(), nx2, pre2.ss)); x = z;
        }
        skips.push_back(x);
      }
      if (i < 3) {
        Tensor y = talloc(x.H / 2, x.W / 2, ch[i], true);
        FusedNorm* nx = pn.offer(m->down_res[i + 1][0].n1, 1e-5f, 1, y.H, y.W, ch[i]);
        GILL_TRY(conv(x, nullptr, m->down_ds[i], 2, 0, nullptr, 0, nullptr, y, nx));
        x = y;
        skips.push_back(x);
      }
    }
    {
      const Handoff::Taken pre = pn.take();
      FusedNorm* nx = pn.offer(m->mid_xf.gn, 1e-6f, 0, x.H, x.W, ch[3]);
      Tensor y; GILL_TRY(resnet(x, nullptr, m->mid_res[0], &y, true, pre.copy(), nx)); x = y;
      const Handoff::Taken pre2 = pn.take();
      FusedNorm* nx2 = pn.offer(m->mid_res[1].n1, 1e-5f, 1, x.H, x.W, ch[3]);
      Tensor z; GILL_TRY(xf(x, m->mid_xf, &z, true, false, pre2.copy(), nx2)); x = z;
      const Handoff::Taken pre3 = pn.take();
      Tensor u; GILL_TRY(resnet(x, nullptr, m->mid_res[1], &u, true, pre3.copy(), nullptr)); x = u;
    }
    for (int i = 0; i < 4; ++i) {
      for (int j = 0; j < 3; ++j) {
        Tensor skip = skips.back(); skips.pop_back();
        Tensor y;
        FusedNorm* nx = (i >= 1) ? pn.offer(m->up_xf[i][j].gn, 1e-6f, 0, x.H, x.W, ch[3 - i], xf_plan_of(m->up_xf[i][j], x.H * x.W, false).gn_table) : nullptr;
        GILL_TRY(resnet(x, &skip, m->up_res[i][j], &y, true, nullptr, nx));
        x = y;
        if (i > 0) {
          const Handoff::Taken pre = pn.take();
          Tensor z; GILL_TRY(xf(x, m->up_xf[i][j], &z, true, false, pre.copy(), nullptr, pre.ss)); x = z;
        }
      }
      if (i < 3) {
        Tensor y = talloc(x.H * 2, x.W * 2, x.C, !m->up_us[i].ups4 || (x.H * x.W) % GN_SLAB_ROWS == 0);
        GILL_TRY(conv(x, nullptr, m->up_us[i], 1, 1, nullptr, 0, nullptr, y));
        x = y;
      }
    }
    Tensor n = talloc(L, L, ch[0]);
    GILL_TRY(gnorm(x, nullptr, m->norm_out, 1e-5f, 1, n));
    GILL_TRY(dbg_sync("last groupnorm"));
    if (!dry) GILL_TRY(conv_out_launch(n.p, m->conv_out_w, m->conv_out_b, Bx, ch[0], L, L, c.out_channels, eps_out, s));
    GILL_TRY(dbg_sync("conv_out"));
    GILL_REQUIRE(dry || m->arena.high <= m->arena.cap, "internal: activation arena overflow (the dry run and the real run allocate differently)");
    return 0;
  }
};

}

static int unet_plan_and_alloc(gill_unet* m) {
  const gill_unet_config& c = m->cfg;
  const int Bx = c.max_batch;
  const int L = c.sample_size;
  const size_t n_lat = (size_t)c.out_channels * L * L, n_in = (size_t)c.in_channels * L * L;
  m->ctx_pad = round_up(c.ctx_len, 64);
  m->arena.dry = true; m->arena.off = 0; m->arena.high = 0;
  m->kcache.assign(m->n_xf, nullptr); m->vcache.assign(m->n_xf, nullptr);
  m->xq_w.assign(m->n_xf, nullptr); m->xo_w.assign(m->n_xf, nullptr); m->xq_cs.assign(m->n_xf, nullptr); m->xq_b.assign(m->n_xf, nullptr);
  UNetRun r{m, nullptr, Bx, nullptr, 0, true};
  GILL_TRY(r.forward(nullptr, nullptr));
  if (Bx % 2 == 0) {
    const size_t gn1 = m->gn_next; const size_t ln1 = m->ln_next; const size_t co1 = m->coop_next;
    r.cfg_pair = true;
    GILL_TRY(r.forward(nullptr, nullptr));
// ... 288 lines not shown
```

### gill_amd/csrc/unet_ops.hip

```cpp
#include "sd_schedule.h"
#include "xf_weights.h"
#include "xf_args.h"

static int op_sd_sampler_run(const gill_sd_sampler* sampler, int v_prediction, int num_steps, int start, float guidance, const float* latents0,
                             const float* init_noise, const float* model_out, const float* noise, int B, int64_t n, float* lat_out,
                             float* unet_in_out, void* stream, int inpaint = 0, const float* latent_mask = nullptr,
                             const float* masked_latents = nullptr, int64_t hw = 0) {
  hipStream_t s = (hipStream_t)stream;
  GILL_REQUIRE(sampler && latents0 && model_out && lat_out && unet_in_out, "null argument");
  GILL_REQUIRE(B >= 1 && n >= 1 && (int64_t)B * n <= ((int64_t)1 << 28), "B, n out of range");
  GILL_REQUIRE(inpaint == 0 || (init_noise && latent_mask && hw >= 1 && n % hw == 0), "inpaint: init_noise, latent_mask and hw dividing n required");
  SdSchedule sched;
  GILL_TRY(sd_schedule(sampler, v_prediction != 0, num_steps, sched, start));
  GILL_REQUIRE(!sched.needs_noise || noise != nullptr, "this sampler draws noise in its steps: a [ncalls][B][n] noise table is required");
  const bool linear = sched.kind != SD_PNDM, cfg = guidance > 1.0f;
  const int ncalls = (int)sched.timesteps.size(), Bx = cfg ? 2 * B : B;
  const size_t total = (size_t)B * n;
  const size_t n_in = inpaint == 2 ? (size_t)(2 * n + hw) : (size_t)n;
  DevBuf rows, ctr, gd, slot, lat, lat2, saved, ring, keepd;
  std::vector<float> keep32;
  if (inpaint == 1) {
    std::vector<double> keep;
    GILL_TRY(sd_inpaint_keep(sampler, v_prediction != 0, num_steps, start, sched, keep));
    keep32.assign(keep.begin(), keep.end());
    GILL_TRY(keepd.alloc(sizeof(float) * keep32.size()));
    GILL_CHECK_HIP(hipMemcpyAsync(keepd.p, keep32.data(), keepd.bytes, hipMemcpyHostToDevice, s));
  }
  GILL_TRY(rows.alloc(linear ? sizeof(SamplerRow) * ncalls : sizeof(PlmsRow) * ncalls));
  GILL_CHECK_HIP(hipMemcpyAsync(rows.p, linear ? (const void*)sched.rows.data() : (const void*)sched.plms.data(), rows.bytes, hipMemcpyHostToDevice, s));
  GILL_TRY(ctr.alloc_zero(sizeof(int) * 2, s));
  GILL_TRY(gd.alloc(sizeof(float)));
  GILL_CHECK_HIP(hipMemcpyAsync(gd.p, &guidance, sizeof(float), hipMemcpyHostToDevice, s));
  GILL_TRY(slot.alloc(sizeof(noise)));
  GILL_CHECK_HIP(hipMemcpyAsync(slot.p, &noise, sizeof(noise), hipMemcpyHostToDevice, s));
  GILL_TRY(lat.alloc(sizeof(float) * total)); GILL_TRY(lat2.alloc(sizeof(float) * (size_t)B * n_in * 2));
  GILL_TRY(saved.alloc(sizeof(float) * total)); GILL_TRY(ring.alloc(sizeof(float) * total * 4));
  GILL_CHECK_HIP(hipStreamSynchronize(s));
  if (init_noise) GILL_TRY(add_noise_f32_launch(latents0, init_noise, (float)sched.add_a, (float)sched.add_b, (int64_t)total, (float*)lat.p, s));
  else GILL_TRY(scale_f32_launch(latents0, (float)sched.init_noise_sigma, (int64_t)total, (float*)lat.p, s));
  SdLoopArgs la;
  la.rows = linear ? nullptr : (const PlmsRow*)rows.p; la.ctr = (int*)ctr.p; la.temb_table = nullptr; la.temb_total = 0; la.temb_cur = nullptr;
  la.lat = (float*)lat.p; la.lat2 = (float*)lat2.p; la.cur_sample = (float*)saved.p; la.ets = (float*)ring.p;
  la.B = B; la.n = n; la.guidance = (const float*)gd.p; la.cfg = cfg ? 1 : 0;
  if (linear) { la.srows = (const SamplerRow*)rows.p; la.noise = (const float* const*)slot.p; }
  SdInpaintArgs ia;
  ia.x0 = latents0; ia.z0 = init_noise; ia.mask = latent_mask; ia.xm = masked_latents; ia.keep = (const float*)keepd.p; ia.hw = hw;
  for (int i = 0; i < ncalls; ++i) {
    ia.l = la;
    GILL_TRY(inpaint == 2 ? sd_stage_concat_launch(ia, s) : sd_stage_launch(la, s));
    const size_t in_floats = inpaint ? (size_t)Bx * n_in : total;
    GILL_CHECK_HIP(hipMemcpyAsync(unet_in_out + (size_t)i * in_floats, lat2.p, sizeof(float) * in_floats, hipMemcpyDeviceToDevice, s));
    la.eps = model_out + (size_t)i * Bx * n;
    GILL_TRY(linear ? sampler_step_launch(la, s) : plms_step_launch(la, s));
    if (inpaint == 1) GILL_TRY(sd_blend_launch(ia, s));
    GILL_CHECK_HIP(hipMemcpyAsync(lat_out + (size_t)i * total, lat.p, sizeof(float) * total, hipMemcpyDeviceToDevice, s));
  }
  GILL_CHECK_HIP(hipStreamSynchronize(s));
  return 0;
}
extern "C" int gill_op_sd_sampler_run(const gill_sd_sampler* sampler, int v_prediction, int num_steps, float guidance, const float* latents0,
                                      const float* model_out, const float* noise, int B, int64_t n, float* lat_out, float* unet_in_out,
                                      void* stream) {
  return op_sd_sampler_run(sampler, v_prediction, num_steps, 0, guidance, latents0, nullptr, model_out, noise, B, n, lat_out, unet_in_out, stream);
}
extern "C" int gill_op_sd_sampler_run_from(const gill_sd_sampler* sampler, int v_prediction, int num_steps, int start, float guidance,
                                           const float* latents0, const float* init_noise, const float* model_out, const float* noise, int B,
                                           int64_t n, float* lat_out, float* unet_in_out, void* stream) {
  GILL_REQUIRE(init_noise != nullptr, "null argument");
  return op_sd_sampler_run(sampler, v_prediction, num_steps, start, guidance, latents0, init_noise, model_out, noise, B, n, lat_out, unet_in_out, stream);
}
extern "C" int gill_op_sd_inpaint_run(const gill_sd_sampler* sampler, int v_prediction, int num_steps, int start, float guidance,
                                      const float* latents0, const float* init_noise, const float* latent_mask, const float* masked_latents,
                                      const float* model_out, const float* noise, int B, int64_t n, int64_t hw, float* lat_out,
                                      float* unet_in_out, void* stream) {
  GILL_REQUIRE(init_noise != nullptr && latent_mask != nullptr, "null argument");
  return op_sd_sampler_run(sampler, v_prediction, num_steps, start, guidance, latents0, init_noise, model_out, noise, B, n, lat_out, unet_in_out,
                           stream, masked_latents ? 2 : 1, latent_mask, masked_latents, hw);
}

extern "C" int gill_op_ffn_fused(const void* t, const float* ln_g, const float* ln_b, const void* W1, const float* b1, const void* W2,
                                 const float* b2, const void* Wp, const float* bp, const void* resid, void* out, float* gn_stats,
                                 int M, int rows_per_batch, const void* o2, const void* Wo, const float* bo2, void* stream) {
  hipStream_t s = (hipStream_t)stream;
  const XfHeads hd = xf_heads(8, 40);
  const int C = 320, inner = 4 * C, heads = hd.heads, d = hd.d, dp = hd.dp, hdp = hd.hdp;
  GILL_REQUIRE(t && ln_g && ln_b && W1 && b1 && W2 && b2 && Wp && bp && resid && out, "null argument");
  GILL_REQUIRE((o2 != nullptr) == (Wo != nullptr) && (o2 != nullptr) == (bo2 != nullptr), "o2 / Wo / bo2: all or none");
  GILL_REQUIRE(ffn_fused_supported(C, M), "ffn_fused: M must be a multiple of 128");
  DevBuf idx, wff1, bff1, sff1, wfo, bfo, w1c, b1c, w2p, st, wpp, o2p, wop;
  if (o2) {
    GILL_TRY(wpp.alloc(sizeof(bf16_t) * (size_t)C * C));
    GILL_TRY(o2p.alloc_zero(sizeof(bf16_t) * (size_t)M * hdp, s));
    GILL_TRY(wop.alloc_zero(sizeof(bf16_t) * (size_t)C * hdp, s));
    GILL_TRY(pad_head_cols_launch(o2, 0, M, heads, d, dp, (bf16_t*)o2p.p, s));
    GILL_TRY(pad_head_cols_launch(Wo, 0, C, heads, d, dp, (bf16_t*)wop.p, s));
  }
  GILL_TRY(idx.alloc(sizeof(int32_t) * 2 * inner));
  GILL_TRY(wff1.alloc(sizeof(bf16_t) * (size_t)2 * inner * C)); GILL_TRY(bff1.alloc(sizeof(float) * 2 * inner)); GILL_TRY(sff1.alloc(sizeof(float) * 2 * inner));
  GILL_TRY(xf_geglu_weights((const bf16_t*)W1, b1, inner, C, ln_g, ln_b, (int32_t*)idx.p, (bf16_t*)wff1.p, (float*)bff1.p, (float*)sff1.p, s));
  GILL_TRY(wfo.alloc(sizeof(bf16_t) * (size_t)C * 5 * C)); GILL_TRY(bfo.alloc(sizeof(float) * C));
  GILL_TRY(xf_ffo_weights(Wp, 0, W2, 0, b2, 1, bp, 1, C, (bf16_t*)wfo.p, (float*)bfo.p, s));
  GILL_TRY(w1c.alloc(sizeof(bf16_t) * (size_t)8 * C * C)); GILL_TRY(b1c.alloc(sizeof(float) * 8 * C)); GILL_TRY(w2p.alloc(sizeof(bf16_t) * (size_t)4 * C * C));
  GILL_TRY(ffn_relayout_launch((const bf16_t*)wff1.p, (const float*)bff1.p, (const bf16_t*)wfo.p, (bf16_t*)w1c.p, (float*)b1c.p,
                               (bf16_t*)w2p.p, o2 ? (bf16_t*)wpp.p : nullptr, s));
  GILL_TRY(st.alloc(sizeof(float) * (size_t)M * 2));
  GILL_TRY(row_sums_launch((const bf16_t*)t, M, C, (float*)st.p, s));
  FfnArgs fa;
  fa.M = M; fa.T = (const bf16_t*)t; fa.ln_stats = (const float*)st.p; fa.ln_planes = 1;
  fa.W1c = (const bf16_t*)w1c.p; fa.b1c = (const float*)b1c.p; fa.W2p = (const bf16_t*)w2p.p;
  fa.Wfo = (const bf16_t*)wfo.p; fa.bo = (const float*)bfo.p; fa.resid = (const bf16_t*)resid; fa.out = (bf16_t*)out;
  fa.gn_stats = gn_stats; fa.rows_per_batch = rows_per_batch;
  if (o2) { fa.X = (const bf16_t*)o2p.p; fa.Wo = (const bf16_t*)wop.p; fa.bo2 = bo2; fa.Wpp = (const bf16_t*)wpp.p; }
  for (int r = 0, rep = op_repeat(); r < rep; ++r) GILL_TRY(ffn_fused_launch(fa, s));
  GILL_CHECK_HIP(hipStreamSynchronize(s));
  return 0;
}

extern "C" int gill_op_geglu_fp8(const void* t, const float* ln_g, const float* ln_b, const void* W, const float* b, void* out, int M, int inner, int C,
                                 void* stream) {
  hipStream_t s = (hipStream_t)stream;
  GILL_REQUIRE(t && ln_g && ln_b && W && b && out && M > 0 && inner % 16 == 0 && C % 128 == 0, "geglu_fp8: null argument / inner % 16 / C % 128");
  DevBuf idx, wperm, bperm, cs, w8, sc, st, t8;
  GILL_TRY(idx.alloc(sizeof(int32_t) * 2 * inner));
  GILL_TRY(wperm.alloc(sizeof(bf16_t) * (size_t)2 * inner * C)); GILL_TRY(bperm.alloc(sizeof(float) * 2 * inner)); GILL_TRY(cs.alloc(sizeof(float) * 2 * inner));
  GILL_TRY(xf_geglu_weights((const bf16_t*)W, b, inner, C, ln_g, ln_b, (int32_t*)idx.p, (bf16_t*)wperm.p, (float*)bperm.p, (float*)cs.p, s));
  GILL_TRY(w8.alloc((size_t)2 * inner * C)); GILL_TRY(sc.alloc(sizeof(float) * 2 * inner));
  GILL_TRY(linear_weight_quant_fp8_launch((const bf16_t*)wperm.p, 2 * inner, C, F8_LIN_ACT_SCALE, (unsigned char*)w8.p, (float*)sc.p, s));
  GILL_TRY(st.alloc(sizeof(float) * (size_t)M * 2));
  GILL_TRY(row_sums_launch((const bf16_t*)t, M, C, (float*)st.p, s));
  GILL_TRY(t8.alloc((size_t)M * C));
  LinF8Args a;
  a.M = M; a.N = 2 * inner; a.K = C; a.A8 = (const unsigned char*)t8.p; a.W8 = (const unsigned char*)w8.p; a.colscale = (const float*)sc.p;
  a.bias = (const float*)bperm.p; a.C = (bf16_t*)out;
  for (int r = 0, rep = op_repeat(); r < rep; ++r) {
    GILL_TRY(ln_quant_fp8_launch((const bf16_t*)t, M, C, (const float*)st.p, 1, 0, 1e-5f, F8_LIN_ACT_SCALE, (unsigned char*)t8.p, s));
    GILL_TRY(geglu_fp8_launch(a, s));
  }
  GILL_CHECK_HIP(hipStreamSynchronize(s));
  return 0;
}

extern "C" int gill_op_linear_weight_quant_fp8(const void* w_bf16, int N, int K, float act_scale, void* w8, float* colscale, void* stream) {
  hipStream_t s = (hipStream_t)stream;
  GILL_REQUIRE(w_bf16 && w8 && colscale && N > 0 && K > 0 && act_scale > 0.f, "linear_weight_quant_fp8: bad argument");
  GILL_TRY(linear_weight_quant_fp8_launch((const bf16_t*)w_bf16, N, K, act_scale, (unsigned char*)w8, colscale, s));
  GILL_CHECK_HIP(hipStreamSynchronize(s));
  return 0;
}
extern "C" int gill_op_ln_quant_fp8(const void* t_bf16, int M, int C, const float* stats, int planes, int ln_rows, float eps, float act_scale,
                                    void* y8, void* stream) {
  hipStream_t s = (hipStream_t)stream;
  GILL_REQUIRE(t_bf16 && stats && y8 && M > 0 && C > 0 && ln_rows >= 0 && ln_rows <= M && (ln_rows == 0 || M <= 2 * ln_rows) && act_scale > 0.f,
               "ln_quant_fp8: bad argument (rows m >= ln_rows read row m - ln_rows: M <= 2 ln_rows)");
  GILL_TRY(ln_quant_fp8_launch((const bf16_t*)t_bf16, M, C, stats, planes, ln_rows, eps, act_scale, (unsigned char*)y8, s));
  GILL_CHECK_HIP(hipStreamSynchronize(s));
  return 0;
}
extern "C" int gill_op_geglu_fp8_q(const void* x8, const void* w8, const float* colscale, const float* bias, void* out_bf16, int M, int N, int K,
                                   void* stream) {
  hipStream_t s = (hipStream_t)stream;
  GILL_REQUIRE(x8 && w8 && colscale && out_bf16, "geglu_fp8_q: null argument");
  LinF8Args a;
  a.M = M; a.N = N; a.K = K; a.A8 = (const unsigned char*)x8; a.W8 = (const unsigned char*)w8; a.colscale = colscale; a.bias = bias;
  a.C = (bf16_t*)out_bf16;
  for (int r = 0, rep = op_repeat(); r < rep; ++r) GILL_TRY(geglu_fp8_launch(a, s));
  GILL_CHECK_HIP(hipStreamSynchronize(s));
  return 0;
}

extern "C" int gill_op_lnproj(int mode, const void* x, void* t, const void* W1, const float* b1, const float* ln_g, const float* ln_b,
                              const void* W2, void* q, void* k, void* vt, int B, int HW, void* stream) {
  hipStream_t s = (hipStream_t)stream;
  const XfHeads hd = xf_heads(8, 40);
  const int C = 320, heads = hd.heads, d = hd.d, dp = hd.dp, dpv = hd.dpv, hdp = hd.hdp, M = B * HW;
  const int nseg = mode == 0 ? 3 : 1;
  GILL_REQUIRE(mode == 0 || mode == 1, "mode must be 0 or 1");
  GILL_REQUIRE(x && t && W1 && b1 && ln_g && ln_b && W2 && q && (mode == 1 || (k && vt)), "null argument");
  GILL_REQUIRE(lnproj_supported(C, M, heads, dp), "lnproj: B * HW must be a multiple of 128");
  DevBuf xp, w1p, w2, w2p, cs, cb;
  GILL_TRY(w2.alloc_zero(sizeof(bf16_t) * (size_t)nseg * hdp * C, s));
  GILL_TRY(w2p.alloc(sizeof(bf16_t) * (size_t)nseg * hdp * C));
  GILL_TRY(cs.alloc_zero(sizeof(float) * (size_t)nseg * hdp, s)); GILL_TRY(cb.alloc_zero(sizeof(float) * (size_t)nseg * hdp, s));
  HeadRows seg[3];
  for (int sg = 0; sg < nseg; ++sg) seg[sg] = HeadRows{(const bf16_t*)W2 + (size_t)sg * C * C, 0};
  GILL_TRY(xf_qkv_weights(seg, nseg, nullptr, heads, d, dp, C, ln_g, ln_b, (bf16_t*)w2.p, (float*)cs.p, (float*)cb.p, (bf16_t*)w2p.p, s));
  LnProjArgs a;
  a.mode = mode; a.M = M; a.T = (bf16_t*)t; a.b1 = b1; a.W2p = (const bf16_t*)w2p.p; a.c2 = (const float*)cb.p;
  a.Cq = (bf16_t*)q; a.Ck = (bf16_t*)k; a.Cvt = (bf16_t*)vt; a.heads = heads; a.dp = dp; a.dpv = dpv; a.ntok = HW; a.ntok_pad = round_up(HW, 32);
  a.qscale = hd.qscale;
  if (mode == 0) {
    a.X = (const bf16_t*)x; a.W1 = (const bf16_t*)W1;
  } else {
    GILL_TRY(xp.alloc_zero(sizeof(bf16_t) * (size_t)M * hdp, s));
    GILL_TRY(w1p.alloc_zero(sizeof(bf16_t) * (size_t)C * hdp, s));
    GILL_TRY(pad_head_cols_launch(x, 0, M, heads, d, dp, (bf16_t*)xp.p, s));
    GILL_TRY(pad_head_cols_launch(W1, 0, C, heads, d, dp, (bf16_t*)w1p.p, s));
    a.X = (const bf16_t*)xp.p; a.W1 = (const bf16_t*)w1p.p;
  }
  for (int r = 0, rep = op_repeat(); r < rep; ++r) GILL_TRY(lnproj_launch(a, s));
  GILL_CHECK_HIP(hipStreamSynchronize(s));
  return 0;
}

extern "C" int gill_op_cross_attention_folded(const void* t, const float* ln_g, const float* ln_b, const void* Wq, const void* Wk, const void* Wv,
                                              const void* Wo, const float* bo, const void* ctx, void* out, void* P, int B, int HW, int C, int H,
                                              int ctx_len, int E, void* stream) {
  hipStream_t s = (hipStream_t)stream;
  GILL_REQUIRE(t && ln_g && ln_b && Wq && Wk && Wv && Wo && bo && ctx && out, "null argument");
  GILL_REQUIRE(H > 0 && H % 2 == 0 && C % H == 0, "cross_attention_folded: an even number of heads dividing C");
  const int d = C / H, M = B * HW, n80 = 80 * H;
  GILL_REQUIRE(d % 16 == 0 && d >= 80 && d <= 160 && C % 64 == 0 && E % 64 == 0 && ctx_len >= 1 && ctx_len <= 80 && HW % 64 == 0,
               "cross_attention_folded: head dim 80..160 (multiple of 16), C and E multiples of 64, at most 80 context tokens, HW a multiple of 64");
  DevBuf wq, wkv, cs, cq, xg, xgb, T, mq, mcs, mb, wo, st, p;
  GILL_TRY(wq.alloc(sizeof(bf16_t) * (size_t)C * C)); GILL_TRY(wkv.alloc(sizeof(bf16_t) * (size_t)2 * C * E));
  GILL_TRY(cs.alloc(sizeof(float) * C)); GILL_TRY(cq.alloc_zero(sizeof(float) * C, s));
  const HeadRows sq = {Wq, 0}, skv[2] = {{Wk, 0}, {Wv, 0}};
  GILL_TRY(xf_qkv_weights(&sq, 1, nullptr, H, d, d, C, ln_g, ln_b, (bf16_t*)wq.p, (float*)cs.p, (float*)cq.p, nullptr, s));
  GILL_TRY(xf_qkv_weights(skv, 2, nullptr, H, d, d, E, nullptr, nullptr, (bf16_t*)wkv.p, nullptr, nullptr, nullptr, s));
  GILL_TRY(xg.alloc(sizeof(bf16_t) * (size_t)2 * H * C * E)); GILL_TRY(xgb.alloc(sizeof(float) * (size_t)H * E));
  GILL_TRY(xalg_fold_launch((const bf16_t*)wq.p, (const float*)cq.p, (const bf16_t*)wkv.p, (const bf16_t*)Wo, H, C, d, d, E, (bf16_t*)xg.p, (float*)xgb.p, s));
  GILL_TRY(T.alloc(sizeof(bf16_t) * (size_t)B * ctx_len * 2 * H * C));
  GILL_TRY(mq.alloc(sizeof(bf16_t) * (size_t)B * n80 * C)); GILL_TRY(wo.alloc(sizeof(bf16_t) * (size_t)B * n80 * C));
  GILL_TRY(mcs.alloc(sizeof(float) * (size_t)B * n80)); GILL_TRY(mb.alloc(sizeof(float) * (size_t)B * n80));
  GILL_TRY(xalg_operands_launch((const bf16_t*)ctx, (const bf16_t*)xg.p, (const float*)xgb.p, B, H, C, E, ctx_len, (bf16_t*)T.p, (bf16_t*)mq.p,
                                (float*)mcs.p, (float*)mb.p, (bf16_t*)wo.p, s));
  GILL_TRY(st.alloc(sizeof(float) * (size_t)M * 2));
  GILL_TRY(row_sums_launch((const bf16_t*)t, M, C, (float*)st.p, s));
  void* pp = P;
  if (!pp) { GILL_TRY(p.alloc(sizeof(bf16_t) * (size_t)M * n80)); pp = p.p; }
  GemmArgs g, g2;
  xf_xalg_args((const bf16_t*)t, M, HW, C, H, {(const float*)st.p, 1, 0}, (const bf16_t*)mq.p, (const float*)mcs.p, (const float*)mb.p, (const bf16_t*)wo.p,
               bo, pp, t, out, &g, &g2);
  for (int r = 0, rep = op_repeat(); r < rep; ++r) { GILL_TRY(gemm_launch(g, s)); GILL_TRY(gemm_launch(g2, s)); }
  GILL_CHECK_HIP(hipStreamSynchronize(s));
  return 0;
}

static int op_ln_splitk(GemmArgs& g, int splitk, DevBuf& ws) {
  g.splitk = splitk > 0 ? splitk : gemm_pick_splitk(g.M, g.N, g.K, g.act, true, false);
  if (g.splitk > 1) {
    GILL_TRY(ws.alloc(sizeof(float) * (size_t)g.splitk * g.M * g.N));
    g.ws = (float*)ws.p;
  }
  return 0;
}
extern "C" int gill_op_linear_rowstats(const void* A, const void* A2, int K1, const void* W, const float* bias, const void* resid, void* T,
                                       float* planes, int planes_cap, int* nplanes, int M, int N, int K, int splitk, void* stream) {
  hipStream_t s = (hipStream_t)stream;
  GILL_REQUIRE(A && W && T && planes && nplanes && M > 0 && N > 0 && K > 0, "linear_rowstats: null argument");
  GILL_REQUIRE((A2 != nullptr) == (K1 < K) && K1 > 0 && K1 <= K, "linear_rowstats: A2 if and only if K1 < K");
  DevBuf ws;
  GemmArgs g;
  g.M = M; g.N = N; g.K = K; g.K1 = K1; g.A = (const bf16_t*)A; g.lda = K1; g.A2 = (const bf16_t*)A2; g.lda2 = K - K1;
  g.W = (const bf16_t*)W; g.bias = bias; g.resid = resid; g.ldr = N; g.act = ACT_NONE; g.C = T; g.ldc = N;
  GILL_TRY(op_ln_splitk(g, splitk, ws));
  g.row_stats = planes;
  *nplanes = gemm_row_planes(g);
  GILL_REQUIRE(*nplanes <= planes_cap, "linear_rowstats: the planes buffer is too small for this launch");
  for (int r = 0, rep = resid == T ? 1 : op_repeat(); r < rep; ++r) GILL_TRY(gemm_launch(g, s));
  GILL_CHECK_HIP(hipStreamSynchronize(s));
  return 0;
}

extern "C" int gill_op_ln_gemm(int mode, const void* T, const float* planes, int P, int ln_rows, const float* ln_g, const float* ln_b, const void* W,
                               const float* b, void* out, void* q, void* k, void* vt, int M, int C, int inner, int nseg, int heads, int d, int ntok,
                               int splitk, void* stream) {
  hipStream_t s = (hipStream_t)stream;
  GILL_REQUIRE(mode == 0 || mode == 1, "ln_gemm: mode must be 0 (GEGLU) or 1 (QKV)");
// ... 40 lines not shown
```

### gill_amd/csrc/xf_plan.h

```cpp
#pragma once
#include <stdlib.h>

bool ffn_fused_supported(int C, int M);
bool lnproj_supported(int C, int M, int heads, int dp);

struct XfEnv { bool lnproj, xalg, ffn_fused; };
inline const XfEnv& xf_env_default() {
  static const XfEnv env = [] {
    auto on = [](const char* name) { const char* e = getenv(name); return !(e && e[0] == '0'); };
    return XfEnv{on("GILL_UNET_LNPROJ"), on("GILL_UNET_XALG"), on("GILL_UNET_FFN_FUSED")};
  }();
  return env;
}

struct XfGeom { int C, heads, dp, ctx_len, ctx_dim, hw, fp8; };

struct XfForms {
  int lnproj;
  int xalg;
  int ffn_fused;
  int ffn_pre;
  int geglu_fp8;
};
inline XfForms xf_forms(const XfGeom& g, const XfEnv& env) {
  const int H = g.heads, hdp = H * g.dp;
  XfForms f;
  f.lnproj = env.lnproj && lnproj_supported(g.C, 128, H, g.dp);
  f.xalg = env.xalg && H % 2 == 0 && g.ctx_len <= 80 && 80 * H <= hdp && g.dp <= 160 && g.C % 64 == 0 && g.ctx_dim % 64 == 0 && g.hw % 64 == 0;
  f.ffn_fused = env.ffn_fused && ffn_fused_supported(g.C, 128);
  f.ffn_pre = f.ffn_fused && hdp == 384;
  f.geglu_fp8 = g.fp8 && g.C % 128 == 0 && !f.ffn_fused;
  return f;
}
inline bool xf_forms_consistent(const XfForms& f) { return !(f.xalg && (f.lnproj || f.ffn_pre)) && (f.ffn_fused || !f.ffn_pre) && !(f.geglu_fp8 && f.ffn_fused); }

enum { XF_CROSS_ATTN = 0, XF_CROSS_XALG = 1 };
enum { XF_FFN_GEMM = 0, XF_FFN_GEMM_FP8 = 1, XF_FFN_FUSED = 2, XF_FFN_FUSED_PRE = 3 };

struct XfPlan {
  int lnproj;
  int gn_table;
  int cross;
  int ffn;
  int M, M1;
};
inline XfPlan xf_plan(const XfForms& f, const XfGeom& g, int Bx_full, int HW, bool shared) {
  XfPlan p;
  p.M = Bx_full * HW;
  p.M1 = shared ? p.M / 2 : p.M;
  p.lnproj = f.lnproj && !shared && lnproj_supported(g.C, p.M, g.heads, g.dp) && HW % 32 == 0;
  p.gn_table = p.lnproj && HW % 128 == 0;
  p.cross = f.xalg ? XF_CROSS_XALG : XF_CROSS_ATTN;
  if (f.ffn_fused && ffn_fused_supported(g.C, p.M) && HW % 128 == 0) p.ffn = f.ffn_pre ? XF_FFN_FUSED_PRE : XF_FFN_FUSED;
  else p.ffn = f.geglu_fp8 ? XF_FFN_GEMM_FP8 : XF_FFN_GEMM;
  return p;
}
```

### gill_amd/ops.py

```python
from __future__ import annotations

import ctypes
from typing import Optional

import torch

from . import _native as N

ACT = {"none": 0, "relu": 1, "gelu": 2, "silu": 3}


def _bf(t: torch.Tensor) -> torch.Tensor:
  assert t.dtype == torch.bfloat16 and t.is_cuda
  return t.contiguous()


def gemm(a: torch.Tensor, w: torch.Tensor, bias: Optional[torch.Tensor] = None, resid: Optional[torch.Tensor] = None,
         alpha: float = 1.0, act: str = "none", out_f32: bool = False, splitk: int = 0, row_major: bool = False, guarded: bool = False):
  if row_major:
    splitk = -1 if splitk <= 1 else -splitk
  a, w = _bf(a), _bf(w)
  M, K = a.shape
  Nn = w.shape[0]
  buf, out = _out_buffer((M, Nn), torch.float32 if out_f32 else torch.bfloat16, a.device, guarded)
# ... 213 lines not shown
def attention_extend_kv8(q: torch.Tensor, k_new: torch.Tensor, v_new: torch.Tensor, K8: torch.Tensor, Vt8: torch.Tensor, Kexp: torch.Tensor,
                         Vexp: torch.Tensor, lens: torch.Tensor, cu_new: torch.Tensor, max_new: int,
                         flags: Optional[torch.Tensor] = None) -> torch.Tensor:
  B, H, pitch, d = _kv8_cache_checks(K8, Vt8, Kexp, Vexp)
  total = q.shape[0]
  ld = q.stride(0)
  for t in (q, k_new, v_new):
    assert t.dtype == torch.bfloat16 and t.is_cuda and tuple(t.shape) == (total, H * d) and t.stride(1) == 1 and t.stride(0) == ld
  assert lens.dtype == torch.int32 and lens.numel() == B and cu_new.dtype == torch.int32 and cu_new.numel() == B + 1
  assert flags is None or (flags.dtype == torch.int32 and flags.numel() == B)
  o = torch.empty((total, H * d), dtype=torch.bfloat16, device=q.device)
  if total == 0:
    return o
  N.check(N.lib().gill_attention_extend_kv8(q.data_ptr(), k_new.data_ptr(), v_new.data_ptr(), ld, N.ptr(K8), N.ptr(Vt8), N.ptr(Kexp),
                                            N.ptr(Vexp), N.ptr(lens), N.ptr(cu_new), N.ptr(o), B, total, int(max_new), H, d, pitch,
                                            N.ptr(flags), N.current_stream()))
  return o


def layernorm(x: torch.Tensor, gamma: torch.Tensor, beta: torch.Tensor, eps: float = 1e-5) -> torch.Tensor:
  assert x.is_cuda and x.dtype in (torch.bfloat16, torch.float32)
  x = x.contiguous()
  Cc = x.shape[-1]
  rows = x.numel() // Cc
  y = torch.empty(x.shape, device=x.device, dtype=torch.bfloat16)
  g, b = gamma.float().contiguous(), beta.float().contiguous()
  N.check(N.lib().gill_op_layernorm(N.ptr(x), int(x.dtype == torch.float32), N.ptr(g), N.ptr(b), N.ptr(y), rows, Cc, eps,
                                    N.current_stream()))
  return y


def groupnorm(x1: torch.Tensor, gamma: torch.Tensor, beta: torch.Tensor, groups: int = 32, eps: float = 1e-5,
              silu: bool = False, x2: Optional[torch.Tensor] = None) -> torch.Tensor:
  x1 = _bf(x1)
  B, H, W, C1 = x1.shape
  C2 = 0
  if x2 is not None:
    x2 = _bf(x2)
    C2 = x2.shape[-1]
  y = torch.empty((B, H, W, C1 + C2), device=x1.device, dtype=torch.bfloat16)
  g, b = gamma.float().contiguous(), beta.float().contiguous()
  N.check(N.lib().gill_op_groupnorm(N.ptr(x1), C1, N.ptr(x2), C2, B, H * W, groups, N.ptr(g), N.ptr(b), eps, int(silu),
                                    N.ptr(y), N.current_stream()))
  return y


GN_SLAB_ROWS_MIN = 16


def _gn_stats_buffer(B: int, rows: int, nbins: int, device) -> torch.Tensor:
  return torch.full((B * (rows // GN_SLAB_ROWS_MIN) * nbins * 2,), float("nan"), device=device, dtype=torch.float32)


def conv3x3_gn_stats(x1: torch.Tensor, w_oihw: torch.Tensor, bin: int, bias: Optional[torch.Tensor] = None, x2: Optional[torch.Tensor] = None,
                     rowvec: Optional[torch.Tensor] = None, resid: Optional[torch.Tensor] = None, xs1: Optional[torch.Tensor] = None,
                     w_sc: Optional[torch.Tensor] = None, xs2: Optional[torch.Tensor] = None, upsample: bool = False, splitk: int = 1):
  x1 = _bf(x1)
  B, IH, IW, C1 = x1.shape
  x2 = None if x2 is None else _bf(x2)
  xs1 = None if xs1 is None else _bf(xs1)
  xs2 = None if xs2 is None else _bf(xs2)
  C2 = 0 if x2 is None else x2.shape[-1]
  CS1 = 0 if xs1 is None else xs1.shape[-1]
  CS2 = 0 if xs2 is None else xs2.shape[-1]
  f = lambda t: None if t is None else t.float().contiguous()
  w, wsc, bias, rowvec = f(w_oihw), f(w_sc), f(bias), f(rowvec)
  Cout = w.shape[0]
  assert w.shape[1] == C1 + C2 and (wsc is None or tuple(wsc.shape) == (Cout, CS1 + CS2))
  resid = None if resid is None else _bf(resid)
  OH, OW = (2 * IH, 2 * IW) if upsample else (IH, IW)
  y = torch.full((B, OH, OW, Cout), float("nan"), device=x1.device, dtype=torch.bfloat16)
  stats = _gn_stats_buffer(B, OH * OW, Cout // bin, x1.device)
  rows, nslab = ctypes.c_int(0), ctypes.c_int(0)
  N.check(N.lib().gill_op_conv3x3_gn_stats(N.ptr(x1), C1, N.ptr(x2), C2, N.ptr(w), N.ptr(bias), N.ptr(rowvec), N.ptr(resid), N.ptr(xs1), CS1,
                                           N.ptr(xs2), CS2, N.ptr(wsc), N.ptr(y), N.ptr(stats), bin, B, IH, IW, Cout, int(upsample), splitk,
                                           ctypes.byref(rows), ctypes.byref(nslab), N.current_stream()))
  return y, stats, rows.value, nslab.value


def gemm_gn_stats(a: torch.Tensor, w: torch.Tensor, bin: int, rows_per_batch: int, bias: Optional[torch.Tensor] = None,
                  resid: Optional[torch.Tensor] = None, splitk: int = 1, act: str = "none"):
  a, w = _bf(a), _bf(w)
  M, K = a.shape
  Nn = w.shape[0]
  bias = None if bias is None else bias.float().contiguous()
  resid = None if resid is None else _bf(resid)
  y = torch.full((M, Nn), float("nan"), device=a.device, dtype=torch.bfloat16)
  stats = _gn_stats_buffer(M // rows_per_batch, rows_per_batch, Nn // bin, a.device)
  rows, nslab = ctypes.c_int(0), ctypes.c_int(0)
  N.check(N.lib().gill_op_gemm_gn_stats(N.ptr(a), N.ptr(w), N.ptr(bias), N.ptr(resid), N.ptr(y), N.ptr(stats), bin, M, Nn, K, rows_per_batch,
                                        splitk, ACT[act], ctypes.byref(rows), ctypes.byref(nslab), N.current_stream()))
  return y, stats, rows.value, nslab.value


def groupnorm_from_stats(x1: torch.Tensor, stats1: torch.Tensor, bin1: int, gamma: torch.Tensor, beta: torch.Tensor, groups: int = 32,
                         eps: float = 1e-5, silu: bool = False, x2: Optional[torch.Tensor] = None, stats2: Optional[torch.Tensor] = None,
                         bin2: int = 0, want_table: bool = False, out8_scale: float = 0.0):
  x1 = _bf(x1)
  B, HW, C1 = x1.shape
  C2 = 0
  if x2 is not None:
    x2 = _bf(x2)
    C2 = x2.shape[-1]
  chk = lambda st, nb: st.is_cuda and st.dtype == torch.float32 and st.is_contiguous() and st.dim() == 4 and st.shape[0] == B and tuple(st.shape[2:]) == (nb, 2)
  assert chk(stats1, C1 // bin1) and (stats2 is None or chk(stats2, C2 // bin2))
  g, b = gamma.float().contiguous(), beta.float().contiguous()
  nan = float("nan")
  y = None if want_table else torch.full((B, HW, C1 + C2), nan, device=x1.device, dtype=torch.bfloat16)
  buf = None
  if out8_scale > 0:
    assert not want_table
    buf, y = _guarded((B, HW, C1 + C2), torch.uint8, x1.device)
  table = torch.full((B, 2, C1 + C2), nan, device=x1.device, dtype=torch.float32) if want_table else None
  N.check(N.lib().gill_op_groupnorm_from_stats(N.ptr(x1), C1, N.ptr(x2), C2, B, HW, groups, N.ptr(g), N.ptr(b), float(eps), int(silu), N.ptr(stats1),
                                               bin1, stats1.shape[1], N.ptr(stats2), bin2, 0 if stats2 is None else stats2.shape[1],
                                               N.ptr(y if buf is None else buf), N.ptr(table), float(out8_scale), N.current_stream()))
  if buf is not None:
    return y, table, stats1, stats2, _guard_ok(buf)
  return y, table, stats1, stats2


def conv3x3_fp8(x: torch.Tensor, w_oihw: torch.Tensor, bias: Optional[torch.Tensor] = None, resid: Optional[torch.Tensor] = None,
                splitk: int = 0) -> torch.Tensor:
  x = _bf(x)
  B, H, W, Cin = x.shape
  w = w_oihw.float().contiguous()
  Cout = w.shape[0]
  assert w.shape[1] == Cin and Cin % 64 == 0
  y = torch.empty((B, H, W, Cout), device=x.device, dtype=torch.bfloat16)
  if bias is not None:
    bias = bias.float().contiguous()
  if resid is not None:
    resid = _bf(resid)
  N.check(N.lib().gill_op_conv3x3_fp8(N.ptr(x), N.ptr(w), N.ptr(bias), N.ptr(resid), N.ptr(y), B, H, W, Cin, Cout, splitk,
                                      N.current_stream()))
  return y


def ffn_fused(t: torch.Tensor, ln_g: torch.Tensor, ln_b: torch.Tensor, w1: torch.Tensor, b1: torch.Tensor, w2: torch.Tensor,
              b2: torch.Tensor, wp: torch.Tensor, bp: torch.Tensor, resid: torch.Tensor, rows_per_batch: int = 0,
              o2: Optional[torch.Tensor] = None, wo: Optional[torch.Tensor] = None, bo2: Optional[torch.Tensor] = None):
  t, w1, w2, wp, resid = (_bf(x) for x in (t, w1, w2, wp, resid))
  M = t.shape[0]
  out = torch.full((M, 320), float("nan"), device=t.device, dtype=torch.bfloat16)
  stats = torch.full((M // 64, 64, 2), float("nan"), device=t.device, dtype=torch.float32) if rows_per_batch else None
  f = lambda x: x.float().contiguous()
  ln_g, ln_b, b1, b2, bp = f(ln_g), f(ln_b), f(b1), f(b2), f(bp)
  if o2 is not None:
    o2, wo, bo2 = _bf(o2), _bf(wo), f(bo2)
  N.check(N.lib().gill_op_ffn_fused(N.ptr(t), N.ptr(ln_g), N.ptr(ln_b), N.ptr(w1), N.ptr(b1), N.ptr(w2), N.ptr(b2), N.ptr(wp), N.ptr(bp),
                                    N.ptr(resid), N.ptr(out), N.ptr(stats), M, rows_per_batch, N.ptr(o2), N.ptr(wo), N.ptr(bo2),
                                    N.current_stream()))
  return (out, stats) if rows_per_batch else out


def lnproj(mode: int, x: torch.Tensor, t, w1: torch.Tensor, b1: torch.Tensor, ln_g: torch.Tensor, ln_b: torch.Tensor, w2: torch.Tensor,
           B: int, HW: int):
  x, w1, w2 = (_bf(v) for v in (x, w1, w2))
  M = B * HW
  hw_pad = (HW + 31) // 32 * 32
  nan = float("nan")
  t = torch.full((M, 320), nan, device=x.device, dtype=torch.bfloat16) if mode == 0 else _bf(t).clone()
  q = torch.full((B, 8, hw_pad, 48), nan, device=x.device, dtype=torch.bfloat16)
  k = torch.full_like(q, nan) if mode == 0 else None
  vt = torch.full((B, 8, 64, hw_pad), nan, device=x.device, dtype=torch.bfloat16) if mode == 0 else None
  f = lambda v: v.float().contiguous()
  b1, ln_g, ln_b = f(b1), f(ln_g), f(ln_b)
  N.check(N.lib().gill_op_lnproj(mode, N.ptr(x), N.ptr(t), N.ptr(w1), N.ptr(b1), N.ptr(ln_g), N.ptr(ln_b), N.ptr(w2), N.ptr(q), N.ptr(k),
                                 N.ptr(vt), B, HW, N.current_stream()))
  return t, q, k, vt


def cross_attention_folded(t: torch.Tensor, ln_g: torch.Tensor, ln_b: torch.Tensor, wq: torch.Tensor, wk: torch.Tensor, wv: torch.Tensor,
                           wo: torch.Tensor, bo: torch.Tensor, ctx: torch.Tensor, heads: int, B: int, HW: int):
  t, wq, wk, wv, wo, ctx = (_bf(v) for v in (t, wq, wk, wv, wo, ctx))
  M, C = t.shape
  E = ctx.shape[-1]
  f = lambda v: v.float().contiguous()
  ln_g, ln_b, bo = f(ln_g), f(ln_b), f(bo)
  nan = float("nan")
  out = torch.full((M, C), nan, device=t.device, dtype=torch.bfloat16)
  P = torch.full((M, 80 * heads), nan, device=t.device, dtype=torch.bfloat16)
  N.check(N.lib().gill_op_cross_attention_folded(N.ptr(t), N.ptr(ln_g), N.ptr(ln_b), N.ptr(wq), N.ptr(wk), N.ptr(wv), N.ptr(wo), N.ptr(bo),
                                                 N.ptr(ctx), N.ptr(out), N.ptr(P), B, HW, C, heads, ctx.shape[1], E, N.current_stream()))
  return out, P


def padded_head_dim(d: int) -> int:
  for dp in (48, 64, 80, 128, 160):
    if d <= dp:
      return dp
  raise ValueError(f"unsupported head dim {d}")


ROWSTATS_GUARD_ROWS = 64


def linear_rowstats(a: torch.Tensor, w: torch.Tensor, bias: Optional[torch.Tensor] = None, resid: Optional[torch.Tensor] = None,
                    a2: Optional[torch.Tensor] = None, splitk: int = 0, inplace: bool = False):
  a, w = _bf(a), _bf(w)
  M, K1 = a.shape
  Nn, K = w.shape
  if a2 is not None:
    a2 = _bf(a2)
    assert a2.shape == (M, K - K1)
  nan = float("nan")
  tbuf = torch.full((M + ROWSTATS_GUARD_ROWS, Nn), nan, device=a.device, dtype=torch.bfloat16)
  if resid is not None:
    resid = _bf(resid)
    if inplace:
      tbuf[:M] = resid
      resid = tbuf
  cap = max((Nn + 63) // 64, 2 * ((Nn + 127) // 128))
  planes = torch.full((cap + 1, M, 2), nan, device=a.device, dtype=torch.float32)
  if bias is not None:
    bias = bias.float().contiguous()
  npl = ctypes.c_int(0)
  N.check(N.lib().gill_op_linear_rowstats(N.ptr(a), N.ptr(a2), K1, N.ptr(w), N.ptr(bias), N.ptr(resid), N.ptr(tbuf), N.ptr(planes), cap,
                                          ctypes.byref(npl), M, Nn, K, splitk, N.current_stream()))
  P = npl.value
  return tbuf[:M], planes[:P], (tbuf[M:], planes[P:])


def ln_gemm_geglu(t: torch.Tensor, planes: torch.Tensor, ln_g: torch.Tensor, ln_b: torch.Tensor, w: torch.Tensor, bias: torch.Tensor,
                  ln_rows: int = 0, splitk: int = 1) -> torch.Tensor:
  t, w = _bf(t), _bf(w)
  M, Cc = t.shape
  inner = w.shape[0] // 2
  planes = planes.float().contiguous()
  assert planes.is_cuda and planes.shape[1:] == (ln_rows or M, 2)
  f = lambda x: x.float().contiguous()
  ln_g, ln_b, bias = f(ln_g), f(ln_b), f(bias)
  out = torch.full((M, inner), float("nan"), device=t.device, dtype=torch.bfloat16)
  N.check(N.lib().gill_op_ln_gemm(0, N.ptr(t), N.ptr(planes), planes.shape[0], ln_rows, N.ptr(ln_g), N.ptr(ln_b), N.ptr(w), N.ptr(bias), N.ptr(out),
                                  None, None, None, M, Cc, inner, 0, 0, 0, 0, splitk, N.current_stream()))
  return out


def ln_gemm_qkv(t: torch.Tensor, planes: Optional[torch.Tensor], ln_g: Optional[torch.Tensor], ln_b: Optional[torch.Tensor], w: torch.Tensor,
                bias: Optional[torch.Tensor], heads: int, ntok: int, ln_rows: int = 0, splitk: int = 1):
  t, w = _bf(t), _bf(w)
  M, Cc = t.shape
  nseg = w.shape[0] // Cc
  d = Cc // heads
  dp = padded_head_dim(d)
  dpv, ntok_pad, B = (dp + 31) // 32 * 32, (ntok + 31) // 32 * 32, M // ntok
  f = lambda x: x.float().contiguous()
  if planes is None:
    assert ln_g is None and ln_b is None
    nplanes = 0
  else:
    planes = planes.float().contiguous()
    assert planes.is_cuda and planes.shape[1:] == (ln_rows or M, 2)
    ln_g, ln_b = f(ln_g), f(ln_b)
    nplanes = planes.shape[0]
  bias = None if bias is None else f(bias)
  nan = float("nan")
  q = torch.full((B, heads, ntok_pad, dp), nan, device=t.device, dtype=torch.bfloat16)
  k = torch.full_like(q, nan) if nseg == 3 else None
  vt = torch.full((B, heads, dpv, ntok_pad), nan, device=t.device, dtype=torch.bfloat16) if nseg == 3 else None
  N.check(N.lib().gill_op_ln_gemm(1, N.ptr(t), N.ptr(planes), nplanes, ln_rows, N.ptr(ln_g), N.ptr(ln_b), N.ptr(w), N.ptr(bias), None,
                                  N.ptr(q), N.ptr(k), N.ptr(vt), M, Cc, 0, nseg, heads, d, ntok, splitk, N.current_stream()))
  return q, k, vt


def sd_sampler_run(sampler, v_prediction: bool, num_steps: int, guidance: float, latents0: torch.Tensor, model_out: torch.Tensor,
                   noise: Optional[torch.Tensor] = None, eta: float = 0.0):
  import ctypes as C
  from .sd import as_sampler_config
  sp = as_sampler_config(sampler).native(eta)
  B, n = latents0.shape
  ncalls = N.lib().gill_sd_schedule(C.byref(sp), int(bool(v_prediction)), int(num_steps), None, None, None)
  if ncalls < 0:
    N.check(ncalls)
  Bx = 2 * B if guidance > 1.0 else B
  if tuple(model_out.shape) != (ncalls, Bx, n) or (noise is not None and tuple(noise.shape) != (ncalls, B, n)):
    raise ValueError(f"model_out must be {(ncalls, Bx, n)} and noise {(ncalls, B, n)}")
  lat0, mo = latents0.float().contiguous(), model_out.float().contiguous()
  z = None if noise is None else noise.float().contiguous()
  lat = torch.empty((ncalls, B, n), device=lat0.device, dtype=torch.float32)
  uin = torch.empty_like(lat)
  N.check(N.lib().gill_op_sd_sampler_run(C.byref(sp), int(bool(v_prediction)), int(num_steps), float(guidance), N.ptr(lat0), N.ptr(mo),
                                         None if z is None else N.ptr(z), B, n, N.ptr(lat), N.ptr(uin), N.current_stream()))
  return lat, uin


def sd_sampler_run_from(sampler, v_prediction: bool, num_steps: int, start: int, guidance: float, latents0: torch.Tensor,
                        init_noise: torch.Tensor, model_out: torch.Tensor, noise: Optional[torch.Tensor] = None, eta: float = 0.0):
  import ctypes as C
  from .sd import as_sampler_config
  sp = as_sampler_config(sampler).native(eta)
  B, n = latents0.shape
  ncalls = N.lib().gill_sd_schedule_from(C.byref(sp), int(bool(v_prediction)), int(num_steps), int(start), None, None, None, None)
  if ncalls < 0:
    N.check(ncalls)
  Bx = 2 * B if guidance > 1.0 else B
  if tuple(model_out.shape) != (ncalls, Bx, n) or (noise is not None and tuple(noise.shape) != (ncalls, B, n)):
    raise ValueError(f"model_out must be {(ncalls, Bx, n)} and noise {(ncalls, B, n)}")
  if tuple(init_noise.shape) != (B, n):
    raise ValueError(f"init_noise must be {(B, n)}")
  lat0, z0, mo = latents0.float().contiguous(), init_noise.float().contiguous(), model_out.float().contiguous()
  z = None if noise is None else noise.float().contiguous()
  lat = torch.empty((ncalls, B, n), device=lat0.device, dtype=torch.float32)
  uin = torch.empty_like(lat)
  N.check(N.lib().gill_op_sd_sampler_run_from(C.byref(sp), int(bool(v_prediction)), int(num_steps), int(start), float(guidance), N.ptr(lat0),
                                              N.ptr(z0), N.ptr(mo), None if z is None else N.ptr(z), B, n, N.ptr(lat), N.ptr(uin),
# ... 540 lines not shown
```

### include/gill_amd.h

```cpp
#ifndef GILL_AMD_H
#define GILL_AMD_H
#include <stdint.h>
#ifdef __cplusplus
extern "C" {
#endif

#define GILL_DTYPE_BF16 0
#define GILL_DTYPE_F32 1
#define GILL_DTYPE_F16 2

typedef struct {
  const char* name;
  const void* data;
  int32_t dtype;
  int32_t ndim;
  int64_t shape[4];
} gill_tensor;

const char* gill_last_error(void);
int gill_version(void);

typedef struct gill_opt gill_opt;
typedef struct {
  int32_t vocab_size;
// ... 161 lines not shown
  int32_t max_positions;
  int32_t hidden_act;
  int32_t max_batch;
} gill_clip_text_config;
typedef struct gill_clip_text gill_clip_text;

int gill_clip_text_create(gill_clip_text** out, const gill_clip_text_config* cfg, const gill_tensor* weights, int n_weights);
void gill_clip_text_destroy(gill_clip_text* h);

int gill_clip_text_forward(gill_clip_text* h, const int32_t* ids, int B, int T, void* out_bf16, float* out_f32, void* stream);

typedef struct gill_mapper gill_mapper;
typedef struct {
  int32_t in_dim;
  int32_t out_dim;
  int32_t hidden_dim;
  int32_t num_heads;
  int32_t ffn_dim;
  int32_t num_enc_layers;
  int32_t num_dec_layers;
  int32_t num_input_tokens;
  int32_t num_output_tokens;
  int32_t max_batch;
} gill_mapper_config;

int gill_mapper_create(gill_mapper** out, const gill_mapper_config* cfg, const gill_tensor* weights, int n_weights);
void gill_mapper_destroy(gill_mapper* h);
int gill_mapper_forward(gill_mapper* h, const void* x_bf16, const void* input_embs_bf16, int B, int Be, float* out,
                        void* stream);

typedef struct gill_unet gill_unet;
typedef struct {
  int32_t in_channels;
  int32_t out_channels;
  int32_t block_out_channels[4];
  int32_t layers_per_block;
  int32_t cross_attention_dim;
  int32_t num_heads;
  int32_t norm_num_groups;
  int32_t sample_size;
  int32_t ctx_len;
  int32_t max_batch;
  int32_t heads_per_level[4];
  int32_t v_prediction;
  int32_t fp8_convs;
} gill_unet_config;

int gill_unet_create(gill_unet** out, const gill_unet_config* cfg, const gill_tensor* weights, int n_weights);
void gill_unet_destroy(gill_unet* h);

int gill_unet_forward(gill_unet* h, const float* sample, const float* timesteps_host, const void* ctx_bf16, int Bx,
                      float* eps_out, void* stream);

int gill_sd_denoise(gill_unet* h, const void* cond_bf16, const void* uncond_bf16, int n_uncond, const float* latents0, int B,
                    int num_steps, float guidance, float* latents_out, void* stream);

typedef struct {
  int32_t kind;
  int32_t steps_offset;
  int32_t set_alpha_to_one;
  float eta;
} gill_sd_sampler;

int gill_sd_denoise_ex(gill_unet* h, const gill_sd_sampler* sampler, const void* cond_bf16, const void* uncond_bf16, int n_uncond,
                       const float* latents0, int B, int num_steps, float guidance, float* latents_out, const float* noise, void* stream);

#define GILL_SD_ROW_DOUBLES 12
int gill_sd_schedule(const gill_sd_sampler* sampler, int v_prediction, int num_steps, float* timesteps_out, double* init_noise_sigma_out,
                     double* rows_out);

int gill_sd_schedule_from(const gill_sd_sampler* sampler, int v_prediction, int num_steps, int start, float* timesteps_out,
                          double* init_noise_sigma_out, double* rows_out, double* add_noise_out);
int gill_sd_denoise_from(gill_unet* h, const gill_sd_sampler* sampler, const void* cond_bf16, const void* uncond_bf16, int n_uncond,
                         int start, const float* init_latents, const float* init_noise, int B, int num_steps, float guidance,
                         float* latents_out, const float* noise, void* stream);

int gill_sd_inpaint_prepare(const float* image, const float* mask, int B, int Bm, int H, int W, float* masked_image_out, float* latent_mask_out,
                            void* stream);
int gill_sd_inpaint_keep(const gill_sd_sampler* sampler, int v_prediction, int num_steps, int start, double* keep_out);
int gill_sd_inpaint(gill_unet* h, const gill_sd_sampler* sampler, const void* cond_bf16, const void* uncond_bf16, int n_uncond, int start,
                    const float* init_latents, const float* init_noise, const float* latent_mask, const float* masked_latents, int B,
                    int num_steps, float guidance, float* latents_out, const float* noise, void* stream);

typedef struct gill_vae gill_vae;
typedef struct {
  int32_t latent_channels;
  int32_t out_channels;
  int32_t block_out_channels[4];
  int32_t layers_per_block;
  int32_t norm_num_groups;
  int32_t latent_size;
  float scaling_factor;
  int32_t max_batch;
} gill_vae_config;

int gill_vae_create(gill_vae** out, const gill_vae_config* cfg, const gill_tensor* weights, int n_weights);
void gill_vae_destroy(gill_vae* h);
int gill_vae_decode(gill_vae* h, const float* latents, int B, float* image_f32, uint8_t* image_u8, void* stream);
int gill_vae_encode(gill_vae* h, const float* image, int B, const float* noise, float* latents_out, float* moments_out, void* stream);

typedef struct gill_ret_index gill_ret_index;

int gill_ret_index_create(gill_ret_index** out, int dim, int64_t capacity);
void gill_ret_index_destroy(gill_ret_index* h);
int gill_ret_index_add(gill_ret_index* h, const void* rows, int dtype, int64_t n, int normalize, float scale, void* stream);
int64_t gill_ret_index_size(const gill_ret_index* h);
int gill_ret_index_rows(gill_ret_index* h, int64_t first, int64_t n, void* out_bf16, void* stream);
int gill_ret_index_search(gill_ret_index* h, const float* queries, int Q, int normalize, int k, const int64_t* exclude, int E, float penalty,
                          float* scores_out, int64_t* idx_out, void* stream);
int gill_ret_index_slabs(const gill_ret_index* h, int64_t* first_row, int* nlists, int64_t* rows_per_list);

int gill_pndm_schedule(int num_steps, int32_t* timesteps_out, double* alphas_cumprod_out);
int gill_coop_timeouts(void);

int gill_op_gemm(const void* A, const void* W, const float* bias, const void* resid, void* C, int M, int N, int K,
                 float alpha, int act, int out_f32, int splitk, void* stream);
int gill_op_geglu(const void* A, const void* W, const float* bias, void* C, int M, int inner, int K, void* stream);
int gill_op_conv3x3(const void* x1, int C1, const void* x2, int C2, const float* w_oihw, const float* bias,
                    const float* rowvec, const void* resid, void* y, int B, int IH, int IW, int Cout, int stride, int ups,
                    int splitk, void* stream);
int gill_op_conv3x3_ex(const void* x1, int C1, const void* x2, int C2, const float* w_oihw, const float* bias,
                       const float* rowvec, const void* resid, void* y, int B, int IH, int IW, int Cout, int stride, int ups,
                       int pad_shift, int splitk, void* stream);
int gill_op_conv3x3_gn(const void* x, const float* w_oihw, const float* bias, const float* rowvec, const void* resid, const float* gamma,
                       const float* beta, int groups, float eps, int silu, void* y_raw, void* y_norm, float* ss_out, int B, int H, int W,
                       int Cin, int Cout, int splitk, int coop, void* stream);
int gill_op_conv3x3_shortcut(const void* x1, int C1, const void* x2, int C2, const float* w_oihw, const float* bias,
                             const void* xs1, int CS1, const void* xs2, int CS2, const float* w_sc, void* y, int B, int IH, int IW,
                             int Cout, int splitk, void* stream);
int gill_op_attention(const void* q, const void* k, const void* v, void* o, int B, int H, int nq, int nkv, int d,
                      float scale, int causal, void* stream);
int gill_op_layernorm(const void* x, int x_f32, const float* gamma, const float* beta, void* y_bf16, int rows, int C,
                      float eps, void* stream);
int gill_op_groupnorm(const void* x1, int C1, const void* x2, int C2, int B, int HW, int groups, const float* gamma,
                      const float* beta, float eps, int silu, void* y, void* stream);

int gill_op_conv3x3_gn_stats(const void* x1, int C1, const void* x2, int C2, const float* w_oihw, const float* bias, const float* rowvec,
                             const void* resid, const void* xs1, int CS1, const void* xs2, int CS2, const float* w_sc, void* y, float* gn_stats,
                             int bin, int B, int IH, int IW, int Cout, int ups, int splitk, int* slab_rows, int* nslab, void* stream);
int gill_op_gemm_gn_stats(const void* A_bf16, const void* W_bf16, const float* bias, const void* resid_bf16, void* C_bf16, float* gn_stats, int bin,
                          int M, int N, int K, int rows_per_batch, int splitk, int act, int* slab_rows, int* nslab, void* stream);
int gill_op_groupnorm_from_stats(const void* x1, int C1, const void* x2, int C2, int B, int HW, int groups, const float* gamma, const float* beta,
                                 float eps, int silu, const float* stats1, int bin1, int nslab1, const float* stats2, int bin2, int nslab2,
                                 void* y, float* ss_out, float out8_scale, void* stream);

int gill_op_vae_attention(const void* n_bf16, const void* resid_bf16, const void* wqkv_bf16, const float* bqkv, const void* wo_bf16,
                          const float* bo, void* out_bf16, void* P_out_bf16, int B, int HW, int C, int* splits, void* stream);
int gill_op_row_softmax(void* s_bf16, int rows, int n, void* stream);

int gill_op_ffn_fused(const void* t_bf16, const float* ln_g, const float* ln_b, const void* W1_bf16, const float* b1,
                      const void* W2_bf16, const float* b2, const void* Wp_bf16, const float* bp, const void* resid_bf16,
                      void* out_bf16, float* gn_stats, int M, int rows_per_batch, const void* o2_bf16, const void* Wo_bf16,
                      const float* bo2, void* stream);

int gill_op_geglu_fp8(const void* t, const float* ln_g, const float* ln_b, const void* W, const float* b, void* out, int M, int inner, int C,
                      void* stream);
int gill_op_lnproj(int mode, const void* x_bf16, void* t_bf16, const void* W1_bf16, const float* b1, const float* ln_g, const float* ln_b,
                   const void* W2_bf16, void* q_bf16, void* k_bf16, void* vt_bf16, int B, int HW, void* stream);

int gill_op_cross_attention_folded(const void* t_bf16, const float* ln_g, const float* ln_b, const void* Wq_bf16, const void* Wk_bf16,
                                   const void* Wv_bf16, const void* Wo_bf16, const float* bo, const void* ctx_bf16, void* out_bf16,
                                   void* P_bf16, int B, int HW, int C, int H, int ctx_len, int E, void* stream);

int gill_op_linear_rowstats(const void* A_bf16, const void* A2_bf16, int K1, const void* W_bf16, const float* bias, const void* resid_bf16,
                            void* T_bf16, float* planes, int planes_cap, int* nplanes, int M, int N, int K, int splitk, void* stream);
int gill_op_ln_gemm(int mode, const void* T_bf16, const float* planes, int P, int ln_rows, const float* ln_g, const float* ln_b, const void* W_bf16,
                    const float* b, void* out_bf16, void* q_bf16, void* k_bf16, void* vt_bf16, int M, int C, int inner, int nseg, int heads, int d,
                    int ntok, int splitk, void* stream);

int gill_op_conv3x3_fp8(const void* x_bf16, const float* w_oihw, const float* bias, const void* resid_bf16, void* y_bf16,
                        int B, int H, int W, int Cin, int Cout, int splitk, void* stream);

int gill_conv_fp8_kpad(int Cin);
int gill_op_quant_fp8(const void* x_bf16, float scale, int64_t n, void* y8, void* stream);
int gill_op_conv_weight_quant_fp8(const void* w_oihw, int dtype, int Cout, int Cin, float act_scale, void* w8, float* colscale, void* stream);
int gill_op_conv3x3_fp8_q(const void* x8, const void* w8, const float* colscale, const float* bias, const float* rowvec, const void* resid_bf16,
                          void* y_bf16, float* gn_stats, int stats_bin, float* ws, int partials_only, int B, int H, int W, int Cin, int Cout,
                          int splitk, void* stream);
int gill_op_groupnorm_fp8(const void* x1, int C1, const void* x2, int C2, int B, int HW, int groups, const float* gamma, const float* beta,
                          float eps, int silu, float scale, void* y8, void* stream);
int gill_op_linear_weight_quant_fp8(const void* w_bf16, int N, int K, float act_scale, void* w8, float* colscale, void* stream);
int gill_op_ln_quant_fp8(const void* t_bf16, int M, int C, const float* stats, int planes, int ln_rows, float eps, float act_scale, void* y8,
                         void* stream);
int gill_op_geglu_fp8_q(const void* x8, const void* w8, const float* colscale, const float* bias, void* out_bf16, int M, int N, int K,
                        void* stream);

int gill_op_sd_sampler_run(const gill_sd_sampler* sampler, int v_prediction, int num_steps, float guidance, const float* latents0,
                           const float* model_out, const float* noise, int B, int64_t n, float* lat_out, float* unet_in_out, void* stream);
int gill_op_sd_sampler_run_from(const gill_sd_sampler* sampler, int v_prediction, int num_steps, int start, float guidance,
                                const float* latents0, const float* init_noise, const float* model_out, const float* noise, int B, int64_t n,
                                float* lat_out, float* unet_in_out, void* stream);
int gill_op_sd_inpaint_run(const gill_sd_sampler* sampler, int v_prediction, int num_steps, int start, float guidance, const float* latents0,
                           const float* init_noise, const float* latent_mask, const float* masked_latents, const float* model_out,
                           const float* noise, int B, int64_t n, int64_t hw, float* lat_out, float* unet_in_out, void* stream);

int gill_op_conv_out(const void* x_bf16, const void* w_oihw, int w_dtype, const float* bias, float* y_f32, int B, int H, int W, int Cin, int Cout,
                     int force_general, int* path, void* stream);
int gill_op_conv_in(const float* x_f32, const void* w_oihw, int w_dtype, const float* bias, void* y_bf16, int B, int Cin, int H, int W, int Cout,
                    uint32_t* counters, int ncounters, void* stream);
int gill_op_conv_in_wide(const float* x_f32, const void* w_oihw, int w_dtype, const float* bias, void* y_bf16, int B, int Cin, int H, int W, int Cout,
                         uint32_t* counters, int ncounters, void* stream);
int gill_op_timestep_embed(const float* t, int n, int dim, void* out_bf16, void* stream);
int gill_op_reduce_ln(const float* ws, int sk, int M, int D, const float* bias, float* h, const float* g, const float* b, void* nb_bf16, float eps,
                      void* stream);
int gill_op_linear_reduce_ln(const void* A_bf16, const void* W_bf16, const float* bias, float* h, const float* g, const float* b, void* nb_bf16,
                             int M, int N, int K, int splitk, int fuse, void* stream);
int gill_op_skinny_gemm(const void* x_bf16, const void* W_bf16, float* out_f32, int M, int N, int K, void* stream);

int gill_op_lm_head_loss(const void* X_bf16, const void* W_bf16, const int64_t* target, int M, int V, int D, float* lse, float* tgt,
                         int32_t* rank, float* summary, void* stream);
int gill_lm_loss_geometry(int M, int V, int D, int* row_tile, int* col_tile, int* n_slabs, int* cols_per_slab);

int gill_op_img_block_heads(const float* hidden_f32, int64_t rows, int D, const int32_t* row_idx, int n, const void* Wr_bf16, const float* br,
                            int E, const void* Wd_bf16, const float* bd, int C, float* ret_emb, float* probs, int32_t* choice, void* stream);
int gill_op_img_rerank_scores(const float* visual_f32, const float* ret_emb_f32, int n, int g, int E, float* scores, void* stream);

#define GILL_GEMM_PLAN_CASE_INTS 54
#define GILL_GEMM_PLAN_ROW_INTS 34
int gill_gemm_plan(const int32_t* cases, int n, int pp, int coop, int cus, int32_t* rows);
int gill_gemm_plan_log(int32_t* rows, int cap, int* launched);
int gill_gemm_query(const int32_t* queries, int n, int pp, int coop, int cus, int32_t* answers);

#define GILL_UNET_XF_PLAN_CASE_INTS 8
#define GILL_UNET_XF_PLAN_ROW_INTS 11
int gill_unet_xf_plan(const int32_t* cases, int n, int lnproj, int xalg, int ffn_fused, int32_t* rows);

#define GILL_ATTENTION_PLAN_INTS 4
int gill_attention_plan(int B, int H, int nq, int nkv, int d, int causal, int att_dma, int32_t* out);

int gill_opt_forward_loss(gill_opt* h, const int64_t* ids, const int32_t* last_idx_host, int B, int T, int num_tokens,
                          const void* extra_rows_bf16, int n_extra, const int64_t* labels, void* raw_out_bf16, void* emb_out_bf16,
                          float* token_loss, int32_t* token_rank, float* summary, float* last_logit_out, float* hidden_out, void* stream);


#ifdef __cplusplus
}
#endif
#endif
```

Before: 8.913.

## Fuse cross-attention into the fused feed-forward kernel ahead of attn2.to_out

```diff
diff --git a/gill_amd/_native.py b/gill_amd/_native.py
--- a/gill_amd/_native.py
+++ b/gill_amd/_native.py
@@ -171,6 +171,7 @@
   "gill_op_conv3x3_gn": (_i, [_vp, _vp, _vp, _vp, _vp, _vp, _vp, _i, _f, _i, _vp, _vp, _vp, _i, _i, _i, _i, _i, _i, _i, _vp]),
   "gill_op_conv3x3_shortcut": (_i, [_vp, _i, _vp, _i, _vp, _vp, _vp, _i, _vp, _i, _vp, _vp, _i, _i, _i, _i, _i, _vp]),
   "gill_op_ffn_fused": (_i, [_vp, _vp, _vp, _vp, _vp, _vp, _vp, _vp, _vp, _vp, _vp, _vp, _i, _i, _vp, _vp, _vp, _vp]),
+  "gill_op_ffn_xattn": (_i, [_vp, _vp, _vp, _vp, _vp, _vp, _vp, _vp, _vp, _vp, _vp, _vp, _i, _i, _vp, _vp, _vp, _i, _i, _vp, _vp, _i, _vp]),
   "gill_op_geglu_fp8": (_i, [_vp, _vp, _vp, _vp, _vp, _vp, _i, _i, _i, _vp]),
   "gill_conv_fp8_kpad": (_i, [_i]),
   "gill_op_quant_fp8": (_i, [_vp, _f, C.c_int64, _vp, _vp]),
diff --git a/gill_amd/csrc/ffn.hip b/gill_amd/csrc/ffn.hip
--- a/gill_amd/csrc/ffn.hip
+++ b/gill_amd/csrc/ffn.hip
@@ -17,6 +17,13 @@
 static_assert(FSMEM_PRE <= 160 * 1024, "LDS budget");
 constexpr int FKO = 384;
 constexpr int FNPRE = 2 * (FKO / 64);
+constexpr int XA_KEYS = 96;
+constexpr int XA_KROW = 96, XA_KHEAD = XA_KEYS * XA_KROW, XA_KPIECE = 8 * XA_KHEAD / 1024;
+constexpr int XA_VROW = 208, XA_VROWS = 41, XA_VHEAD = XA_VROWS * XA_VROW, XA_V_OFF = XA_KPIECE * 1024;
+constexpr int XA_VPIECE = (8 * XA_VHEAD + 1023) / 1024, XA_NPIECE = XA_KPIECE + XA_VPIECE;
+constexpr int XA_ZERO_OFF = FBO2_OFF + FC * 4;
+constexpr int FSMEM_XA = XA_ZERO_OFF + 16;
+static_assert(8 * XA_KHEAD == XA_KPIECE * 1024 && XA_NPIECE * 1024 <= FBIAS_OFF && FSMEM_XA <= 160 * 1024, "attention images inside the ring");
 
 typedef __attribute__((ext_vector_type(16))) float f32x16;
 typedef __attribute__((ext_vector_type(4))) float f32x4;
@@ -29,8 +36,9 @@
 
 struct Slab { const bf16_t* src; int ld; };
 
-template <bool PRE>
+template <bool PRE, bool XA = false>
 __global__ __launch_bounds__(256) __attribute__((amdgpu_waves_per_eu(1, 1))) void ffn_fused_kernel(const FfnArgs p) {
+  static_assert(PRE || !XA, "the cross-attention feeds attn2.to_out");
   kernarg_warm<sizeof(FfnArgs)>();
   constexpr int SB = PRE ? FNPRE % 7 : 0;
   extern __shared__ __attribute__((aligned(16))) unsigned char smem[];
@@ -63,26 +71,74 @@
     return *reinterpret_cast<const bf16x8*>(slot + row * 128 + (((2 * s + hi) ^ (row & 7)) * 16));
   };
 
-#pragma unroll
-  for (int f = 0; f < 6; ++f) {
-    const Slab st = PRE ? slab_g(f) : slab_f(f);
-#pragma unroll
-    for (int i = 0; i < 5; ++i) issue_piece(st, f, i);
+  auto issue_first6 = [&]() {
+#pragma unroll
+    for (int f = 0; f < 6; ++f) {
+      const Slab st = PRE ? slab_g(f) : slab_f(f);
+#pragma unroll
+      for (int i = 0; i < 5; ++i) issue_piece(st, f, i);
+    }
+  };
+  int xa_b = 0, xa_nk16 = 0;
+  if constexpr (XA) {
+    xa_b = __builtin_amdgcn_readfirstlane((blockIdx.x * FTM) / p.x_hw);
+    xa_nk16 = __builtin_amdgcn_readfirstlane((p.x_ctx_len + 15) >> 4);
+    const int nkp = 16 * xa_nk16;
+    const int kvb = p.x_kv_bstride_zero ? 0 : xa_b;
+    const char* Kb = (const char*)(p.XK + (size_t)kvb * 8 * p.x_nkv_pad * 48);
+    const char* Vb = (const char*)(p.XVt + (size_t)kvb * 8 * p.x_dpv * p.x_nkv_pad);
+    for (int pc = w; pc < XA_NPIECE; pc += 4) {
+      unsigned off;
+      const char* base;
+      if (pc < XA_KPIECE) {
+        const int c = pc * 64 + lane;
+        const int head = c / (XA_KHEAD / 16), r = c - head * (XA_KHEAD / 16);
+        int key = r / 6;
+        const int ch = r - key * 6;
+        key = key < nkp ? key : 0;
+        off = (unsigned)(((head * p.x_nkv_pad + key) * 48 + ch * 8) * 2);
+        base = Kb;
+      } else {
+        const int c = (pc - XA_KPIECE) * 64 + lane;
+        int head = c / (XA_VHEAD / 16);
+        const int r = c - head * (XA_VHEAD / 16);
+        head = head < 8 ? head : 7;
+        const int row = r / 13;
+        int ch = r - row * 13;
+        ch = 8 * ch < nkp ? ch : 0;
+        const int vrow = row == 40 ? 48 : row;
+        off = (unsigned)(((head * p.x_dpv + vrow) * p.x_nkv_pad + ch * 8) * 2);
+        base = Vb;
+      }
+      __builtin_amdgcn_global_load_lds((const __attribute__((address_space(1))) void*)(base + off),
+                                       (__attribute__((address_space(3))) void*)(smem + pc * 1024), 16, 0, 0);
+    }
+  } else {
+    issue_first6();
   }
   __builtin_amdgcn_sched_barrier(0);
   bf16x8 tf[20];
   float ln_mean, ln_rstd;
   bf16x8 xf[PRE ? FKO / 16 : 1];
   u32x4 res[PRE ? 20 : 1];
-  if constexpr (PRE) {
+  auto load_res = [&]() {
     const bf16_t* tsrc = p.T + (size_t)(blockIdx.x * FTM + w * 32 + (lane >> 2)) * FC + (lane & 3) * 8;
 #pragma unroll
     for (int i = 0; i < 10; ++i) {
       res[2 * i] = *reinterpret_cast<const u32x4*>(tsrc + 32 * i);
       res[2 * i + 1] = *reinterpret_cast<const u32x4*>(tsrc + 32 * i + 16 * FC);
     }
-#pragma unroll
-    for (int s = 0; s < FKO / 16; ++s) xf[s] = *reinterpret_cast<const bf16x8*>(p.X + (size_t)m * FKO + 16 * s + 8 * hi);
+  };
+  if constexpr (PRE) {
+    if constexpr (!XA) load_res();
+    if constexpr (XA) {
+      const bf16_t* qsrc = p.XQ + ((size_t)xa_b * 8 * p.x_nq_pad + (m - xa_b * p.x_hw)) * 48 + 8 * hi;
+#pragma unroll
+      for (int s = 0; s < FKO / 16; ++s) xf[s] = *reinterpret_cast<const bf16x8*>(qsrc + (size_t)(s / 3) * p.x_nq_pad * 48 + 16 * (s % 3));
+    } else {
+#pragma unroll
+      for (int s = 0; s < FKO / 16; ++s) xf[s] = *reinterpret_cast<const bf16x8*>(p.X + (size_t)m * FKO + 16 * s + 8 * hi);
+    }
   } else {
 #pragma unroll
     for (int s = 0; s < 20; ++s) tf[s] = *reinterpret_cast<const bf16x8*>(p.T + (size_t)m * FC + 16 * s + 8 * hi);
@@ -111,6 +167,9 @@
       float* b2t = reinterpret_cast<float*>(smem + FBO2_OFF);
       const float v0 = p.bo2[tid], v1 = p.bo2[min(tid + 256, FC - 1)];
       b2t[tid] = v0; b2t[min(tid + 256, FC - 1)] = v1;
+    }
+    if constexpr (XA) {
+      if (tid < 4) *reinterpret_cast<unsigned*>(smem + XA_ZERO_OFF + 4 * tid) = 0u;
     }
   }
 
@@ -157,8 +216,94 @@
 
   __builtin_amdgcn_s_waitcnt(0xC07F);
   __builtin_amdgcn_s_barrier();
-#pragma unroll
-  for (int q = 0; q < 5; ++q) wf[0][q] = wfrag(smem, q, 0);
+  if constexpr (XA) {
+    const float NEG_INF = -__builtin_inff();
+    const int ctx_len = p.x_ctx_len;
+    const int sw = (l31 & ~12) | ((l31 & 4) << 1) | ((l31 & 8) >> 1);
+    const unsigned char* kfr = smem + sw * XA_KROW + hi * 16;
+    const unsigned char* vfr0 = smem + XA_V_OFF + sw * XA_VROW + hi * 16;
+    const unsigned char* vfr1 = smem + XA_V_OFF + min(32 + sw, 40) * XA_VROW + hi * 16;
+    const f32x16 zero16 = {0, 0, 0, 0, 0, 0, 0, 0, 0, 0, 0, 0, 0, 0, 0, 0};
+    auto attend = [&](auto nk_tag) {
+      constexpr int NK = decltype(nk_tag)::value;
+      auto has = [&](int u) { return NK ? u < NK : u < xa_nk16; };
+      auto scores = [&](int h, f32x16* sc) {
+#pragma unroll
+        for (int t = 0; t < 3; ++t) {
+          if (has(2 * t)) {
+            const unsigned char* kt = kfr + h * XA_KHEAD + t * 32 * XA_KROW;
+            const unsigned char* k2 = hi ? smem + XA_ZERO_OFF : kt + 64;
+            sc[t] = __builtin_amdgcn_mfma_f32_32x32x16_bf16(*reinterpret_cast<const bf16x8*>(kt), xf[3 * h], zero16, 0, 0, 0);
+            sc[t] = __builtin_amdgcn_mfma_f32_32x32x16_bf16(*reinterpret_cast<const bf16x8*>(kt + 32), xf[3 * h + 1], sc[t], 0, 0, 0);
+            sc[t] = __builtin_amdgcn_mfma_f32_32x32x16_bf16(*reinterpret_cast<const bf16x8*>(k2), xf[3 * h + 2], sc[t], 0, 0, 0);
+          }
+        }
+      };
+      f32x16 scs[2][3];
+      scores(0, scs[0]);
+#pragma unroll
+      for (int h = 0; h < 8; ++h) {
+        if (h + 1 < 8) scores(h + 1, scs[(h + 1) & 1]);
+        f32x16* sc = scs[h & 1];
+        float mx = NEG_INF;
+#pragma unroll
+        for (int u = 0; u < 6; ++u) {
+          if (has(u)) {
+            const int t = u >> 1, r0 = 8 * (u & 1);
+            if (NK ? u == NK - 1 : 16 * u + 16 > ctx_len) {
+#pragma unroll
+              for (int j = 0; j < 8; ++j) sc[t][r0 + j] = (16 * u + 8 * hi + j >= ctx_len) ? NEG_INF : sc[t][r0 + j];
+            }
+#pragma unroll
+            for (int j = 0; j < 8; ++j) mx = fmaxf(mx, sc[t][r0 + j]);
+          }
+        }
+        mx = fmaxf(mx, __shfl_xor(mx, 32, 64));
+        bf16x8 pf[6];
+#pragma unroll
+        for (int u = 0; u < 6; ++u) {
+          if (has(u)) {
+            union { bf16x8 v; unsigned u[4]; } pk;
+#pragma unroll
+            for (int j = 0; j < 4; ++j)
+              pk.u[j] = pack_bf2(__builtin_amdgcn_exp2f(sc[u >> 1][8 * (u & 1) + 2 * j] - mx), __builtin_amdgcn_exp2f(sc[u >> 1][8 * (u & 1) + 2 * j + 1] - mx));
+            pf[u] = pk.v;
+          }
+        }
+        f32x16 o0 = zero16, o1 = zero16;
+#pragma unroll
+        for (int u = 0; u < 6; ++u) {
+          if (has(u)) {
+            o0 = __builtin_amdgcn_mfma_f32_32x32x16_bf16(*reinterpret_cast<const bf16x8*>(vfr0 + h * XA_VHEAD + u * 32), pf[u], o0, 0, 0, 0);
+            o1 = __builtin_amdgcn_mfma_f32_32x32x16_bf16(*reinterpret_cast<const bf16x8*>(vfr1 + h * XA_VHEAD + u * 32), pf[u], o1, 0, 0, 0);
+          }
+        }
+        const float inv = 1.f / __shfl(o1[0], 32 + l31, 64);
+        union { bf16x8 v; unsigned u[4]; } x0, x1, x2;
+#pragma unroll
+        for (int j = 0; j < 4; ++j) {
+          x0.u[j] = pack_bf2(o0[2 * j] * inv, o0[2 * j + 1] * inv);
+          x1.u[j] = pack_bf2(o0[8 + 2 * j] * inv, o0[8 + 2 * j + 1] * inv);
+          x2.u[j] = hi ? 0u : pack_bf2(o1[2 * j] * inv, o1[2 * j + 1] * inv);
+        }
+        xf[3 * h] = x0.v; xf[3 * h + 1] = x1.v; xf[3 * h + 2] = x2.v;
+        __builtin_amdgcn_sched_barrier(0);
+      }
+    };
+    if (xa_nk16 == 5) attend(std::integral_constant<int, 5>{});
+    else attend(std::integral_constant<int, 0>{});
+    asm volatile("s_waitcnt lgkmcnt(0)" ::: "memory");
+    __builtin_amdgcn_sched_barrier(0);
+    __builtin_amdgcn_s_barrier();
+    asm volatile("" ::: "memory");
+    load_res();
+    __builtin_amdgcn_sched_barrier(0);
+    issue_first6();
+    __builtin_amdgcn_sched_barrier(0);
+  } else {
+#pragma unroll
+    for (int q = 0; q < 5; ++q) wf[0][q] = wfrag(smem, q, 0);
+  }
 
   if constexpr (PRE) {
     f32x16 acc1[10];
@@ -180,9 +325,14 @@
         }
       }
     }
+    if constexpr (XA) ffn_wait_vm<0>();
     __builtin_amdgcn_s_waitcnt(0xC07F);
     __builtin_amdgcn_s_barrier();
     __builtin_amdgcn_sched_barrier(0);
+    if constexpr (XA) {
+#pragma unroll
+      for (int q = 0; q < 5; ++q) wf[0][q] = wfrag(smem, q, 0);
+    }
 #define G_STAGE(G)                                                                                                               \
     {                                                                                                                            \
       auto mma = [&](int s, const bf16x8* wfp) {                                                                                 \
@@ -407,6 +557,7 @@
 }
 
 bool ffn_fused_supported(int C, int M) { return C == FC && M % FTM == 0 && M > 0; }
+bool ffn_xattn_supported(int heads, int d, int ctx_len, int hw) { return heads == 8 && d == 40 && ctx_len >= 1 && ctx_len <= XA_KEYS && hw > 0 && hw % FTM == 0; }
 
 int ffn_relayout_launch(const bf16_t* wff1, const float* bff1, const bf16_t* wfo, bf16_t* W1c, float* b1c, bf16_t* W2p, bf16_t* Wpp,
                         hipStream_t s) {
@@ -419,20 +570,30 @@
   GILL_REQUIRE(ffn_fused_supported(FC, a.M), "fused feed-forward block: M must be a multiple of 128");
   GILL_REQUIRE(a.T && a.W1c && a.b1c && a.W2p && a.bo && a.resid && a.out, "fused feed-forward block: null operand");
   GILL_REQUIRE(!a.gn_stats || (a.rows_per_batch > 0 && a.rows_per_batch % 128 == 0), "fused feed-forward block: GroupNorm partials need whole 64-row slabs per sample");
-  const bool pre = a.X != nullptr;
+  const bool xa = a.XQ != nullptr;
+  const bool pre = a.X != nullptr || xa;
+  if (xa) {
+    GILL_REQUIRE(!a.X && a.XK && a.XVt, "fused feed-forward block with the cross-attention in front: K / V^T missing, or both X and XQ given");
+    GILL_REQUIRE(ffn_xattn_supported(8, 40, a.x_ctx_len, a.x_hw) && a.M % a.x_hw == 0, "fused feed-forward block with the cross-attention in front: 1..96 keys, whole 128-row tiles per sample");
+    GILL_REQUIRE(a.x_nq_pad >= a.x_hw && a.x_nkv_pad % 8 == 0 && a.x_nkv_pad >= round_up(a.x_ctx_len, 16) && a.x_dpv > 48,
+                 "fused feed-forward block with the cross-attention in front: operand padding too small");
+    GILL_REQUIRE(((uintptr_t)a.XQ | (uintptr_t)a.XK | (uintptr_t)a.XVt) % 16 == 0, "fused feed-forward block with the cross-attention in front: operands must be 16-byte aligned");
+  }
   if (pre) {
     GILL_REQUIRE(a.Wo && a.bo2 && a.Wpp, "fused feed-forward block with attn2.to_out in front: null operand");
   } else {
     GILL_REQUIRE(a.Wfo && a.ln_stats && a.ln_planes >= 1, "fused feed-forward block: LayerNorm row-sum planes missing");
   }
-  static bool attr_set[2] = {false, false};
-  const void* fn = pre ? (const void*)ffn_fused_kernel<true> : (const void*)ffn_fused_kernel<false>;
-  const int smem = pre ? FSMEM_PRE : FSMEM;
-  if (!attr_set[pre]) {
+  static bool attr_set[3] = {false, false, false};
+  const int form = xa ? 2 : pre ? 1 : 0;
+  const void* fn = xa ? (const void*)ffn_fused_kernel<true, true> : pre ? (const void*)ffn_fused_kernel<true> : (const void*)ffn_fused_kernel<false>;
+  const int smem = xa ? FSMEM_XA : pre ? FSMEM_PRE : FSMEM;
+  if (!attr_set[form]) {
     GILL_CHECK_HIP(hipFuncSetAttribute(fn, hipFuncAttributeMaxDynamicSharedMemorySize, smem));
-    attr_set[pre] = true;
-  }
-  if (pre) hipLaunchKernelGGL(ffn_fused_kernel<true>, dim3(a.M / FTM), dim3(256), smem, s, a);
+    attr_set[form] = true;
+  }
+  if (xa) hipLaunchKernelGGL((ffn_fused_kernel<true, true>), dim3(a.M / FTM), dim3(256), smem, s, a);
+  else if (pre) hipLaunchKernelGGL(ffn_fused_kernel<true>, dim3(a.M / FTM), dim3(256), smem, s, a);
   else hipLaunchKernelGGL(ffn_fused_kernel<false>, dim3(a.M / FTM), dim3(256), smem, s, a);
   GILL_CHECK_HIP(hipGetLastError());
   return 0;
diff --git a/gill_amd/csrc/ops.h b/gill_amd/csrc/ops.h
--- a/gill_amd/csrc/ops.h
+++ b/gill_amd/csrc/ops.h
@@ -167,7 +167,10 @@
   const bf16_t* X = nullptr;
   const bf16_t* Wo = nullptr; const float* bo2 = nullptr;
   const bf16_t* Wpp = nullptr;
-};
+  const bf16_t* XQ = nullptr; const bf16_t* XK = nullptr; const bf16_t* XVt = nullptr;
+  int x_hw = 0, x_ctx_len = 0, x_nq_pad = 0, x_nkv_pad = 0, x_dpv = 0, x_kv_bstride_zero = 0;
+};
+bool ffn_xattn_supported(int heads, int d, int ctx_len, int hw);
 bool ffn_fused_supported(int C, int M);
 int ffn_relayout_launch(const bf16_t* wff1, const float* bff1, const bf16_t* wfo, bf16_t* W1c, float* b1c, bf16_t* W2p, bf16_t* Wpp,
                         hipStream_t s);
diff --git a/gill_amd/csrc/unet.hip b/gill_amd/csrc/unet.hip
--- a/gill_amd/csrc/unet.hip
+++ b/gill_amd/csrc/unet.hip
@@ -525,6 +525,7 @@
     bf16_t *q, *k, *vt, *o;
     RowStats st1, st2, st3;
     XfHeads heads() const { return xf_heads(w.heads, w.d); }
+    bool ffn_xattn() const { return xf_ffn_xattn(p, w.geom, xf_env_default()); }
     LnProjArgs lnproj_args() const {
       LnProjArgs lp;
       lp.M = p.M; lp.T = t.p; lp.heads = w.heads; lp.dp = w.dp; lp.dpv = w.dpv; lp.ntok = HW; lp.ntok_pad = hw_pad;
@@ -569,6 +570,7 @@
       GILL_TRY(gemm(g));
     }
     GILL_REQUIRE(m->kcache[w.layer_id] != nullptr || dry, "internal: cross-attention K/V cache missing");
+    if (b.ffn_xattn()) return 0;
     GILL_TRY(attend(b.q, m->kcache[w.layer_id], m->vcache[w.layer_id], b.o, b.HW, m->cfg.ctx_len, b.hw_pad, m->ctx_pad, w));
     if (p.ffn == XF_FFN_FUSED_PRE) return 0;
     return linear(b.o, hdp, nullptr, 0, hdp, p.M, w.out2.w, w.out2.b, C, hdp, b.t.p, ACT_NONE, b.t.p, C, nullptr, &b.st3);
@@ -582,6 +584,10 @@
       fa.M = M; fa.T = b.t.p; fa.ln_stats = b.st3.p; fa.ln_planes = b.st3.planes;
       fa.W1c = w.w1c; fa.b1c = w.b1c; fa.W2p = w.w2p; fa.Wfo = w.wfo; fa.bo = w.bfo; fa.resid = b.xd.p; fa.out = out->p;
       if (p.ffn == XF_FFN_FUSED_PRE) { fa.X = b.o; fa.Wo = w.out2.w; fa.bo2 = w.out2.b; fa.Wpp = w.wpp; }
+      if (b.ffn_xattn()) {
+        fa.X = nullptr; fa.XQ = b.q; fa.XK = m->kcache[w.layer_id]; fa.XVt = m->vcache[w.layer_id];
+        fa.x_hw = b.HW; fa.x_ctx_len = m->cfg.ctx_len; fa.x_nq_pad = b.hw_pad; fa.x_nkv_pad = m->ctx_pad; fa.x_dpv = w.dpv;
+      }
       if (out->stats && out->sbin == 5) { fa.gn_stats = out->stats; fa.rows_per_batch = b.HW; out->nslab = b.HW / GN_SLAB_ROWS; }
       else out->stats = nullptr;
       return ffn_fused_launch(fa, s);
diff --git a/gill_amd/csrc/unet_ops.hip b/gill_amd/csrc/unet_ops.hip
--- a/gill_amd/csrc/unet_ops.hip
+++ b/gill_amd/csrc/unet_ops.hip
@@ -78,21 +78,39 @@
                            stream, masked_latents ? 2 : 1, latent_mask, masked_latents, hw);
 }
 
-extern "C" int gill_op_ffn_fused(const void* t, const float* ln_g, const float* ln_b, const void* W1, const float* b1, const void* W2,
-                                 const float* b2, const void* Wp, const float* bp, const void* resid, void* out, float* gn_stats,
-                                 int M, int rows_per_batch, const void* o2, const void* Wo, const float* bo2, void* stream) {
+static int op_ffn_fused(const void* t, const float* ln_g, const float* ln_b, const void* W1, const float* b1, const void* W2, const float* b2,
+                        const void* Wp, const float* bp, const void* resid, void* out, float* gn_stats, int M, int rows_per_batch,
+                        const void* o2, const void* Wo, const float* bo2, const void* xq, const void* xk, const void* xv, int Bkv, int ctx_len,
+                        int xfused, void* stream) {
   hipStream_t s = (hipStream_t)stream;
   const XfHeads hd = xf_heads(8, 40);
   const int C = 320, inner = 4 * C, heads = hd.heads, d = hd.d, dp = hd.dp, hdp = hd.hdp;
   GILL_REQUIRE(t && ln_g && ln_b && W1 && b1 && W2 && b2 && Wp && bp && resid && out, "null argument");
-  GILL_REQUIRE((o2 != nullptr) == (Wo != nullptr) && (o2 != nullptr) == (bo2 != nullptr), "o2 / Wo / bo2: all or none");
+  const bool pre = o2 != nullptr || xq != nullptr;
+  GILL_REQUIRE(pre == (Wo != nullptr) && pre == (bo2 != nullptr), "o2 / Wo / bo2: all or none");
   GILL_REQUIRE(ffn_fused_supported(C, M), "ffn_fused: M must be a multiple of 128");
-  DevBuf idx, wff1, bff1, sff1, wfo, bfo, w1c, b1c, w2p, st, wpp, o2p, wop;
-  if (o2) {
+  DevBuf idx, wff1, bff1, sff1, wfo, bfo, w1c, b1c, w2p, st, wpp, o2p, wop, Q, K, Vt;
+  AttnArgs at;
+  if (xq) {
+    GILL_REQUIRE(!o2 && xk && xv, "ffn_xattn: xq / xk / xv all or none, and not together with o2");
+    GILL_REQUIRE(ffn_xattn_supported(heads, d, ctx_len, rows_per_batch) && M % rows_per_batch == 0, "ffn_xattn: 1..96 context tokens, whole 128-row tiles per sample");
+    const int B = M / rows_per_batch, nq_pad = round_up(rows_per_batch, 32), nkv_pad = round_up(ctx_len, 64);
+    GILL_REQUIRE(Bkv == B || Bkv == 1, "ffn_xattn: one context per sample, or one for all");
+    GILL_TRY(Q.alloc_zero(sizeof(bf16_t) * (size_t)B * heads * nq_pad * dp, s));
+    GILL_TRY(K.alloc_zero(sizeof(bf16_t) * (size_t)Bkv * heads * nkv_pad * dp, s));
+    GILL_TRY(Vt.alloc_zero(sizeof(bf16_t) * (size_t)Bkv * heads * hd.dpv * nkv_pad, s));
+    GILL_TRY(pack_heads_launch((const bf16_t*)xq, B, rows_per_batch, heads, d, nq_pad, dp, hd.dpv, 0, (bf16_t*)Q.p, s, hd.qscale));
+    GILL_TRY(pack_heads_launch((const bf16_t*)xk, Bkv, ctx_len, heads, d, nkv_pad, dp, hd.dpv, 0, (bf16_t*)K.p, s));
+    GILL_TRY(pack_heads_launch((const bf16_t*)xv, Bkv, ctx_len, heads, d, nkv_pad, dp, hd.dpv, 1, (bf16_t*)Vt.p, s));
+    at.Q = (const bf16_t*)Q.p; at.K = (const bf16_t*)K.p; at.Vt = (const bf16_t*)Vt.p;
+    at.B = B; at.H = heads; at.nq = rows_per_batch; at.nkv = ctx_len; at.nq_pad = nq_pad; at.nkv_pad = nkv_pad; at.dp = dp; at.dpv = hd.dpv;
+    at.ldo = hdp; at.d = d; at.scale = 1.0f / sqrtf((float)d); at.kv_bstride_zero = (Bkv == 1 && B > 1) ? 1 : 0;
+  }
+  if (pre) {
     GILL_TRY(wpp.alloc(sizeof(bf16_t) * (size_t)C * C));
     GILL_TRY(o2p.alloc_zero(sizeof(bf16_t) * (size_t)M * hdp, s));
     GILL_TRY(wop.alloc_zero(sizeof(bf16_t) * (size_t)C * hdp, s));
-    GILL_TRY(pad_head_cols_launch(o2, 0, M, heads, d, dp, (bf16_t*)o2p.p, s));
+    if (o2) GILL_TRY(pad_head_cols_launch(o2, 0, M, heads, d, dp, (bf16_t*)o2p.p, s));
     GILL_TRY(pad_head_cols_launch(Wo, 0, C, heads, d, dp, (bf16_t*)wop.p, s));
   }
   GILL_TRY(idx.alloc(sizeof(int32_t) * 2 * inner));
@@ -102,7 +120,7 @@
   GILL_TRY(xf_ffo_weights(Wp, 0, W2, 0, b2, 1, bp, 1, C, (bf16_t*)wfo.p, (float*)bfo.p, s));
   GILL_TRY(w1c.alloc(sizeof(bf16_t) * (size_t)8 * C * C)); GILL_TRY(b1c.alloc(sizeof(float) * 8 * C)); GILL_TRY(w2p.alloc(sizeof(bf16_t) * (size_t)4 * C * C));
   GILL_TRY(ffn_relayout_launch((const bf16_t*)wff1.p, (const float*)bff1.p, (const bf16_t*)wfo.p, (bf16_t*)w1c.p, (float*)b1c.p,
-                               (bf16_t*)w2p.p, o2 ? (bf16_t*)wpp.p : nullptr, s));
+                               (bf16_t*)w2p.p, pre ? (bf16_t*)wpp.p : nullptr, s));
   GILL_TRY(st.alloc(sizeof(float) * (size_t)M * 2));
   GILL_TRY(row_sums_launch((const bf16_t*)t, M, C, (float*)st.p, s));
   FfnArgs fa;
@@ -110,10 +128,32 @@
   fa.W1c = (const bf16_t*)w1c.p; fa.b1c = (const float*)b1c.p; fa.W2p = (const bf16_t*)w2p.p;
   fa.Wfo = (const bf16_t*)wfo.p; fa.bo = (const float*)bfo.p; fa.resid = (const bf16_t*)resid; fa.out = (bf16_t*)out;
   fa.gn_stats = gn_stats; fa.rows_per_batch = rows_per_batch;
-  if (o2) { fa.X = (const bf16_t*)o2p.p; fa.Wo = (const bf16_t*)wop.p; fa.bo2 = bo2; fa.Wpp = (const bf16_t*)wpp.p; }
-  for (int r = 0, rep = op_repeat(); r < rep; ++r) GILL_TRY(ffn_fused_launch(fa, s));
-  GILL_CHECK_HIP(hipStreamSynchronize(s));
-  return 0;
+  if (pre) { fa.X = (const bf16_t*)o2p.p; fa.Wo = (const bf16_t*)wop.p; fa.bo2 = bo2; fa.Wpp = (const bf16_t*)wpp.p; }
+  if (xq && xfused) {
+    fa.X = nullptr; fa.XQ = at.Q; fa.XK = at.K; fa.XVt = at.Vt;
+    fa.x_hw = rows_per_batch; fa.x_ctx_len = ctx_len; fa.x_nq_pad = at.nq_pad; fa.x_nkv_pad = at.nkv_pad; fa.x_dpv = at.dpv;
+    fa.x_kv_bstride_zero = at.kv_bstride_zero;
+  }
+  for (int r = 0, rep = op_repeat(); r < rep; ++r) {
+    if (xq && !xfused) { at.O = (bf16_t*)o2p.p; GILL_TRY(attention_launch(at, s)); }
+    GILL_TRY(ffn_fused_launch(fa, s));
+  }
+  GILL_CHECK_HIP(hipStreamSynchronize(s));
+  return 0;
+}
+extern "C" int gill_op_ffn_fused(const void* t, const float* ln_g, const float* ln_b, const void* W1, const float* b1, const void* W2,
+                                 const float* b2, const void* Wp, const float* bp, const void* resid, void* out, float* gn_stats,
+                                 int M, int rows_per_batch, const void* o2, const void* Wo, const float* bo2, void* stream) {
+  return op_ffn_fused(t, ln_g, ln_b, W1, b1, W2, b2, Wp, bp, resid, out, gn_stats, M, rows_per_batch, o2, Wo, bo2, nullptr, nullptr, nullptr, 0, 0, 0,
+                      stream);
+}
+extern "C" int gill_op_ffn_xattn(const void* t, const float* ln_g, const float* ln_b, const void* W1, const float* b1, const void* W2,
+                                 const float* b2, const void* Wp, const float* bp, const void* resid, void* out, float* gn_stats,
+                                 int M, int rows_per_batch, const void* xq, const void* xk, const void* xv, int Bkv, int ctx_len,
+                                 const void* Wo, const float* bo2, int fused, void* stream) {
+  GILL_REQUIRE(xq && xk && xv && Wo && bo2, "ffn_xattn: null argument");
+  return op_ffn_fused(t, ln_g, ln_b, W1, b1, W2, b2, Wp, bp, resid, out, gn_stats, M, rows_per_batch, nullptr, Wo, bo2, xq, xk, xv, Bkv, ctx_len,
+                      fused ? 1 : 0, stream);
 }
 
 extern "C" int gill_op_geglu_fp8(const void* t, const float* ln_g, const float* ln_b, const void* W, const float* b, void* out, int M, int inner, int C,
diff --git a/gill_amd/csrc/xf_plan.h b/gill_amd/csrc/xf_plan.h
--- a/gill_amd/csrc/xf_plan.h
+++ b/gill_amd/csrc/xf_plan.h
@@ -4,11 +4,11 @@
 bool ffn_fused_supported(int C, int M);
 bool lnproj_supported(int C, int M, int heads, int dp);
 
-struct XfEnv { bool lnproj, xalg, ffn_fused; };
+struct XfEnv { bool lnproj, xalg, ffn_fused; bool ffn_xattn = false; };
 inline const XfEnv& xf_env_default() {
   static const XfEnv env = [] {
     auto on = [](const char* name) { const char* e = getenv(name); return !(e && e[0] == '0'); };
-    return XfEnv{on("GILL_UNET_LNPROJ"), on("GILL_UNET_XALG"), on("GILL_UNET_FFN_FUSED")};
+    return XfEnv{on("GILL_UNET_LNPROJ"), on("GILL_UNET_XALG"), on("GILL_UNET_FFN_FUSED"), on("GILL_UNET_FFN_XATTN")};
   }();
   return env;
 }
@@ -55,3 +55,6 @@
   else p.ffn = f.geglu_fp8 ? XF_FFN_GEMM_FP8 : XF_FFN_GEMM;
   return p;
 }
+inline bool xf_ffn_xattn(const XfPlan& p, const XfGeom& g, const XfEnv& env) {
+  return env.ffn_xattn && p.ffn == XF_FFN_FUSED_PRE && p.cross == XF_CROSS_ATTN && g.heads == 8 && g.C == 320 && g.dp == 48 && g.ctx_len >= 1 && g.ctx_len <= 96;
+}
diff --git a/gill_amd/ops.py b/gill_amd/ops.py
--- a/gill_amd/ops.py
+++ b/gill_amd/ops.py
@@ -389,6 +389,22 @@
                                     N.ptr(resid), N.ptr(out), N.ptr(stats), M, rows_per_batch, N.ptr(o2), N.ptr(wo), N.ptr(bo2),
                                     N.current_stream()))
   return (out, stats) if rows_per_batch else out
+
+
+def ffn_xattn(t: torch.Tensor, ln_g: torch.Tensor, ln_b: torch.Tensor, w1: torch.Tensor, b1: torch.Tensor, w2: torch.Tensor,
+              b2: torch.Tensor, wp: torch.Tensor, bp: torch.Tensor, resid: torch.Tensor, rows_per_batch: int, q: torch.Tensor,
+              k: torch.Tensor, v: torch.Tensor, wo: torch.Tensor, bo2: torch.Tensor, fused: bool = True):
+  t, w1, w2, wp, resid, q, k, v, wo = (_bf(x) for x in (t, w1, w2, wp, resid, q, k, v, wo))
+  M = t.shape[0]
+  assert q.shape == (M, 320) and k.dim() == 3 and k.shape == v.shape and k.shape[2] == 320, "q (M, 320); k, v (Bkv, ctx_len, 320)"
+  out = torch.full((M, 320), float("nan"), device=t.device, dtype=torch.bfloat16)
+  stats = torch.full((M // 64, 64, 2), float("nan"), device=t.device, dtype=torch.float32)
+  f = lambda x: x.float().contiguous()
+  ln_g, ln_b, b1, b2, bp, bo2 = f(ln_g), f(ln_b), f(b1), f(b2), f(bp), f(bo2)
+  N.check(N.lib().gill_op_ffn_xattn(N.ptr(t), N.ptr(ln_g), N.ptr(ln_b), N.ptr(w1), N.ptr(b1), N.ptr(w2), N.ptr(b2), N.ptr(wp), N.ptr(bp),
+                                    N.ptr(resid), N.ptr(out), N.ptr(stats), M, rows_per_batch, N.ptr(q), N.ptr(k), N.ptr(v), k.shape[0],
+                                    k.shape[1], N.ptr(wo), N.ptr(bo2), int(bool(fused)), N.current_stream()))
+  return out, stats
 
 
 def lnproj(mode: int, x: torch.Tensor, t, w1: torch.Tensor, b1: torch.Tensor, ln_g: torch.Tensor, ln_b: torch.Tensor, w2: torch.Tensor,
diff --git a/include/gill_amd.h b/include/gill_amd.h
--- a/include/gill_amd.h
+++ b/include/gill_amd.h
@@ -337,6 +337,10 @@
                       const void* W2_bf16, const float* b2, const void* Wp_bf16, const float* bp, const void* resid_bf16,
                       void* out_bf16, float* gn_stats, int M, int rows_per_batch, const void* o2_bf16, const void* Wo_bf16,
                       const float* bo2, void* stream);
+int gill_op_ffn_xattn(const void* t_bf16, const float* ln_g, const float* ln_b, const void* W1_bf16, const float* b1,
+                      const void* W2_bf16, const float* b2, const void* Wp_bf16, const float* bp, const void* resid_bf16,
+                      void* out_bf16, float* gn_stats, int M, int rows_per_batch, const void* xq_bf16, const void* xk_bf16,
+                      const void* xv_bf16, int Bkv, int ctx_len, const void* Wo_bf16, const float* bo2, int fused, void* stream);
 
 int gill_op_geglu_fp8(const void* t, const float* ln_g, const float* ln_b, const void* W, const float* b, void* out, int M, int inner, int C,
                       void* stream);
```

Result: no change. 8.953, median of 6 (+0.4%).
